# robertknight/rten

Measured on NVIDIA H100. Metric: resnet50_fp32_inferences_per_sec, higher is better.
Workload: dtype f32(tf32 mma, explicit opt-in)

## Files before the change

include/rten_b200.h:

```cpp
#ifndef RTEN_B200_H
#define RTEN_B200_H

#include <stddef.h>
#include <stdint.h>

#ifdef __cplusplus
extern "C" {
#endif

#define RTEN_MAX_DIMS 8
#define RTEN_DEVICE_HOST (-1)

typedef enum { RTEN_F32 = 0, RTEN_I32 = 1, RTEN_I8 = 2, RTEN_U8 = 3 } rten_dtype;

typedef struct {
    void* data;
    int32_t dtype;
    int32_t ndim;
    int64_t shape[RTEN_MAX_DIMS];
    int64_t strides[RTEN_MAX_DIMS];
    int32_t device;
    int32_t _reserved;
} rten_tensor;

// ... 37 lines not shown
rten_status rten_b200_ctx_create(int device, void* cuda_stream_or_null, size_t workspace_bytes, rten_ctx** out);
void rten_b200_ctx_destroy(rten_ctx* ctx);
const char* rten_b200_last_error(rten_ctx* ctx);
rten_status rten_b200_sync(rten_ctx* ctx);
rten_status rten_b200_set_f32_mode(rten_ctx* ctx, int mode );
rten_status rten_b200_set_autotune(rten_ctx* ctx, int enable);
rten_status rten_b200_save_plans(rten_ctx* ctx, const char* path);
rten_status rten_b200_load_plans(rten_ctx* ctx, const char* path);
rten_status rten_b200_alloc(rten_ctx* ctx, size_t bytes, void** dev_ptr);
rten_status rten_b200_free(rten_ctx* ctx, void* dev_ptr);
rten_status rten_b200_host_alloc(rten_ctx* ctx, size_t bytes, void** host_ptr);
rten_status rten_b200_host_free(rten_ctx* ctx, void* host_ptr);
rten_status rten_b200_copy(rten_ctx* ctx, const rten_tensor* src, rten_tensor* dst);
uint64_t rten_b200_launch_count(rten_ctx* ctx);
const char* rten_b200_version(void);
rten_status rten_b200_debug_forced_plans(rten_ctx* ctx, uint64_t* matched, uint64_t* unmatched);
typedef struct rten_graph rten_graph;
rten_status rten_b200_graph_begin(rten_ctx* ctx);
rten_status rten_b200_graph_end(rten_ctx* ctx, rten_graph** out);
rten_status rten_b200_graph_launch(rten_ctx* ctx, rten_graph* g);
void rten_b200_graph_destroy(rten_graph* g);

rten_status rten_b200_prepack_b(rten_ctx* ctx, const rten_tensor* b, rten_packed** out);
rten_status rten_b200_prepack_conv_weight(rten_ctx* ctx, const rten_tensor* w, int groups, rten_packed** out);
void rten_b200_packed_free(rten_ctx* ctx, rten_packed* p);

rten_status rten_b200_gemm(rten_ctx* ctx, const rten_tensor* a, const rten_tensor* b, const rten_tensor* c_or_null,
                           float alpha, float beta, int trans_a, int trans_b, rten_tensor* out);

rten_status rten_b200_matmul(rten_ctx* ctx, const rten_tensor* a, const rten_tensor* b,
                             const rten_packed* packed_b_or_null, const rten_tensor* row_bias_or_null, float alpha,
                             rten_tensor* out);
rten_status rten_b200_matmul_ex(rten_ctx* ctx, const rten_tensor* a, const rten_tensor* b,
                                const rten_packed* packed_b_or_null, const rten_tensor* row_bias_or_null, float alpha,
                                const rten_tensor* residual_or_null, int activation, rten_tensor* out);

rten_status rten_b200_matmul_integer(rten_ctx* ctx, const rten_tensor* a, const rten_tensor* b,
                                     const rten_packed* packed_b_or_null, const rten_tensor* a_zero_point_or_null,
                                     const rten_tensor* b_zero_point_or_null, const rten_tensor* scale_or_null,
                                     rten_tensor* out);
rten_status rten_b200_matmul_integer_ex(rten_ctx* ctx, const rten_tensor* a, const rten_tensor* b, const rten_packed* packed_b,
                                        const rten_tensor* a_zero_point, const rten_tensor* b_zero_point,
                                        const rten_tensor* scale, const rten_tensor* scale_b_or_null ,
                                        const rten_tensor* bias, const rten_tensor* residual, int activation,
                                        rten_tensor* out_range_or_null, rten_tensor* out);

rten_status rten_b200_matmul_nbits(rten_ctx* ctx, const rten_tensor* a, const rten_tensor* b, const rten_tensor* scales,
                                   int bits, int block_size, rten_tensor* out);

typedef struct {
    int32_t pads[4];
    int32_t auto_pad_same;
    int32_t groups;
    int32_t strides[2];
    int32_t dilations[2];
    int32_t n_strides;
    int32_t n_dilations;
} rten_conv_params;
rten_status rten_b200_conv2d(rten_ctx* ctx, const rten_tensor* x, const rten_tensor* w,
                             const rten_packed* packed_w_or_null, const rten_tensor* bias_or_null,
                             const rten_conv_params* p, rten_tensor* out);
rten_status rten_b200_conv2d_ex(rten_ctx* ctx, const rten_tensor* x, const rten_tensor* w,
                                const rten_packed* packed_w_or_null, const rten_tensor* bias_or_null,
                                const rten_conv_params* p, const rten_tensor* residual_or_null, int activation,
                                rten_tensor* out);
rten_status rten_b200_conv2d_act(rten_ctx* ctx, const rten_tensor* x, const rten_tensor* w,
                                 const rten_packed* packed_w_or_null, const rten_tensor* bias_or_null,
                                 const rten_conv_params* p, const rten_tensor* residual_or_null,
                                 const rten_activation* act_or_null, rten_tensor* out);
rten_status rten_b200_conv2d_projected(rten_ctx* ctx, const rten_tensor* x, const rten_tensor* w,
                                       const rten_packed* packed_w_or_null, const rten_tensor* bias_or_null,
                                       const rten_conv_params* p, const rten_tensor* x_proj, const rten_tensor* w_proj,
                                       const rten_packed* packed_w_proj_or_null, const rten_tensor* bias_proj_or_null,
                                       const rten_conv_params* p_proj, int activation, rten_tensor* out);
rten_status rten_b200_conv2d_chained(rten_ctx* ctx, const rten_tensor* x, const rten_tensor* w,
                                     const rten_packed* packed_w_or_null, const rten_tensor* bias_or_null,
                                     const rten_conv_params* p, const rten_tensor* residual_or_null,
                                     const rten_tensor* x_proj_or_null, const rten_tensor* w_proj_or_null,
                                     const rten_packed* packed_w_proj_or_null, const rten_tensor* bias_proj_or_null,
                                     const rten_conv_params* p_proj_or_null, int activation, const rten_tensor* w_next,
                                     const rten_packed* packed_w_next_or_null, const rten_tensor* bias_next_or_null,
                                     const rten_conv_params* p_next, int activation_next, rten_tensor* out,
                                     rten_tensor* out_next);
typedef struct {
    int32_t pads[4];
    int32_t auto_pad_same;
    int32_t groups;
    int32_t strides[2];
    int32_t dilations[2];
    int32_t output_padding[2];
    int32_t n_pads;
    int32_t n_strides;
    int32_t n_dilations;
    int32_t n_output_padding;
} rten_conv_transpose_params;
rten_status rten_b200_conv_transpose(rten_ctx* ctx, const rten_tensor* x, const rten_tensor* w,
                                     const rten_packed* packed_w_or_null, const rten_tensor* bias_or_null,
                                     const rten_conv_transpose_params* p, rten_tensor* out);
rten_status rten_b200_prepack_conv_transpose_weight(rten_ctx* ctx, const rten_tensor* w, const rten_conv_transpose_params* p,
                                                    rten_packed** out);
rten_status rten_b200_conv_integer(rten_ctx* ctx, const rten_tensor* x, const rten_tensor* w,
                                   const rten_packed* packed_w_or_null, const rten_tensor* x_zero_point_or_null,
                                   const rten_tensor* w_zero_point_or_null, const rten_tensor* scale_or_null,
                                   const rten_conv_params* p, rten_tensor* out);
rten_status rten_b200_conv_integer_ex(rten_ctx* ctx, const rten_tensor* x, const rten_tensor* w, const rten_packed* packed_w,
                                      const rten_tensor* x_zero_point, const rten_tensor* w_zero_point,
                                      const rten_tensor* scale, const rten_tensor* scale_b_or_null,
                                      const rten_conv_params* params, const rten_tensor* bias, const rten_tensor* residual,
                                      int activation, rten_tensor* out_range_or_null, rten_tensor* out);

rten_status rten_b200_quantized_linear(rten_ctx* ctx, const rten_tensor* x, const rten_tensor* ln_scale_or_null,
                                       const rten_tensor* ln_bias_or_null, float ln_epsilon, const rten_tensor* w,
                                       const rten_packed* packed_w_or_null, const rten_tensor* w_zero_point_or_null,
                                       const rten_tensor* w_scale, const rten_tensor* bias_or_null,
                                       const rten_tensor* residual_or_null, int activation, rten_tensor* out);
typedef struct {
    int32_t is_causal;
    int32_t q_num_heads;
    int32_t kv_num_heads;
    float scale;
    float softcap;
} rten_attention_params;
rten_status rten_b200_attention(rten_ctx* ctx, const rten_tensor* query, const rten_tensor* key, const rten_tensor* value,
                                const rten_tensor* attn_mask_or_null, const rten_tensor* nonpad_kv_seqlen_or_null,
                                const rten_attention_params* params, const rten_tensor* new_key_or_null,
                                const rten_tensor* new_value_or_null, rten_tensor* out);

rten_status rten_b200_rotary_embedding(rten_ctx* ctx, const rten_tensor* input, const rten_tensor* cos, const rten_tensor* sin,
                                       const rten_tensor* position_ids_or_null, int interleaved, int num_heads,
                                       int rotary_embedding_dim, rten_tensor* out);

typedef struct {
    int32_t num_heads;
    int32_t kv_num_heads;
    float scale;
    int32_t do_rotary;
    int32_t rotary_interleaved;
    int32_t local_window_size;
    float softcap;
} rten_gqa_params;
rten_status rten_b200_group_query_attention(rten_ctx* ctx, const rten_tensor* query, const rten_tensor* key_or_null,
                                            const rten_tensor* value_or_null, const rten_tensor* past_key_or_null,
                                            const rten_tensor* past_value_or_null, const rten_tensor* seqlens_k,
                                            const rten_tensor* total_sequence_length, const rten_tensor* cos_or_null,
                                            const rten_tensor* sin_or_null, const rten_tensor* position_ids_or_null,
                                            const rten_tensor* attention_bias_or_null, const rten_gqa_params* params,
                                            rten_tensor* out, rten_tensor* present_key, rten_tensor* present_value);

typedef struct {
    int32_t num_heads;
    float scale;
    float mask_filter_value;
    int32_t unidirectional;
} rten_mha_params;
rten_status rten_b200_multi_head_attention(rten_ctx* ctx, const rten_tensor* query, const rten_tensor* key_or_null,
                                           const rten_tensor* value_or_null, const rten_tensor* bias_or_null,
                                           const rten_tensor* key_padding_mask_or_null, const rten_tensor* attention_bias_or_null,
                                           const rten_tensor* past_key_or_null, const rten_tensor* past_value_or_null,
                                           const rten_tensor* past_sequence_length_or_null, const rten_tensor* cache_indirection_or_null,
                                           const rten_mha_params* params, rten_tensor* out, rten_tensor* present_key_or_null,
                                           rten_tensor* present_value_or_null);

typedef struct {
    int32_t direction;
    int32_t hidden_size;
    int32_t linear_before_reset;
// ... 112 lines not shown
```

rten_b200/_lib.py:

```python
from __future__ import annotations

import ctypes as C
import os

_HERE = os.path.dirname(os.path.abspath(__file__))
LIB_PATH = os.path.join(_HERE, "librten_b200.so")

RTEN_MAX_DIMS = 8
RTEN_DEVICE_HOST = -1
RTEN_F32, RTEN_I32, RTEN_I8, RTEN_U8 = 0, 1, 2, 3

STATUS_NAMES = {
    0: "Ok", 1: "CastFailed", 2: "UnsupportedType", 3: "IncompatibleInputShapes", 4: "MissingInputs",
    5: "InvalidValue", 6: "UnsupportedValue", 7: "UnsupportedOutput", 100: "Cuda", 101: "Nccl",
}


class RtenTensor(C.Structure):
    _fields_ = [
        ("data", C.c_void_p),
        ("dtype", C.c_int32),
        ("ndim", C.c_int32),
        ("shape", C.c_int64 * RTEN_MAX_DIMS),
        ("strides", C.c_int64 * RTEN_MAX_DIMS),
# ... 21 lines not shown
class RtenConvTransposeParams(C.Structure):
    _fields_ = [
        ("pads", C.c_int32 * 4),
        ("auto_pad_same", C.c_int32),
        ("groups", C.c_int32),
        ("strides", C.c_int32 * 2),
        ("dilations", C.c_int32 * 2),
        ("output_padding", C.c_int32 * 2),
        ("n_pads", C.c_int32),
        ("n_strides", C.c_int32),
        ("n_dilations", C.c_int32),
        ("n_output_padding", C.c_int32),
    ]


class RtenAttentionParams(C.Structure):
    _fields_ = [("is_causal", C.c_int32), ("q_num_heads", C.c_int32), ("kv_num_heads", C.c_int32), ("scale", C.c_float),
                ("softcap", C.c_float)]


class RtenGqaParams(C.Structure):
    _fields_ = [("num_heads", C.c_int32), ("kv_num_heads", C.c_int32), ("scale", C.c_float), ("do_rotary", C.c_int32),
                ("rotary_interleaved", C.c_int32), ("local_window_size", C.c_int32), ("softcap", C.c_float)]


class RtenMhaParams(C.Structure):
    _fields_ = [("num_heads", C.c_int32), ("scale", C.c_float), ("mask_filter_value", C.c_float), ("unidirectional", C.c_int32)]


class RtenActivation(C.Structure):
    _fields_ = [("kind", C.c_int32), ("alpha", C.c_float), ("beta", C.c_float)]


class RtenResizeParams(C.Structure):
    _fields_ = [("mode", C.c_int32), ("coord_mode", C.c_int32), ("nearest_mode", C.c_int32), ("n", C.c_int32),
                ("scales", C.c_float * 4), ("sizes", C.c_int64 * 4), ("use_sizes", C.c_int32)]


class RtenRnnParams(C.Structure):
    _fields_ = [("direction", C.c_int32), ("hidden_size", C.c_int32), ("linear_before_reset", C.c_int32)]


_TP = C.POINTER(RtenTensor)
_vp = C.c_void_p

_SIGNATURES = {
    "rten_b200_version": (C.c_char_p, []),
    "rten_b200_ctx_create": (C.c_int, [C.c_int, _vp, C.c_size_t, C.POINTER(_vp)]),
    "rten_b200_ctx_destroy": (None, [_vp]),
    "rten_b200_last_error": (C.c_char_p, [_vp]),
    "rten_b200_sync": (C.c_int, [_vp]),
    "rten_b200_set_f32_mode": (C.c_int, [_vp, C.c_int]),
    "rten_b200_set_autotune": (C.c_int, [_vp, C.c_int]),
    "rten_b200_save_plans": (C.c_int, [_vp, C.c_char_p]),
    "rten_b200_load_plans": (C.c_int, [_vp, C.c_char_p]),
    "rten_b200_alloc": (C.c_int, [_vp, C.c_size_t, C.POINTER(_vp)]),
    "rten_b200_free": (C.c_int, [_vp, _vp]),
    "rten_b200_host_alloc": (C.c_int, [_vp, C.c_size_t, C.POINTER(_vp)]),
    "rten_b200_host_free": (C.c_int, [_vp, _vp]),
    "rten_b200_copy": (C.c_int, [_vp, _TP, _TP]),
    "rten_b200_launch_count": (C.c_uint64, [_vp]),
    "rten_b200_debug_forced_plans": (C.c_int, [_vp, C.POINTER(C.c_uint64), C.POINTER(C.c_uint64)]),
    "rten_b200_graph_begin": (C.c_int, [_vp]),
    "rten_b200_graph_end": (C.c_int, [_vp, C.POINTER(_vp)]),
    "rten_b200_graph_launch": (C.c_int, [_vp, _vp]),
    "rten_b200_graph_destroy": (None, [_vp]),
    "rten_b200_prepack_b": (C.c_int, [_vp, _TP, C.POINTER(_vp)]),
    "rten_b200_prepack_conv_weight": (C.c_int, [_vp, _TP, C.c_int, C.POINTER(_vp)]),
    "rten_b200_packed_free": (None, [_vp, _vp]),
    "rten_b200_gemm": (C.c_int, [_vp, _TP, _TP, _TP, C.c_float, C.c_float, C.c_int, C.c_int, _TP]),
    "rten_b200_matmul": (C.c_int, [_vp, _TP, _TP, _vp, _TP, C.c_float, _TP]),
    "rten_b200_matmul_ex": (C.c_int, [_vp, _TP, _TP, _vp, _TP, C.c_float, _TP, C.c_int, _TP]),
    "rten_b200_matmul_integer": (C.c_int, [_vp, _TP, _TP, _vp, _TP, _TP, _TP, _TP]),
    "rten_b200_matmul_integer_ex": (C.c_int, [_vp, _TP, _TP, _vp, _TP, _TP, _TP, _TP, _TP, _TP, C.c_int, _TP, _TP]),
    "rten_b200_matmul_nbits": (C.c_int, [_vp, _TP, _TP, _TP, C.c_int, C.c_int, _TP]),
    "rten_b200_conv2d": (C.c_int, [_vp, _TP, _TP, _vp, _TP, C.POINTER(RtenConvParams), _TP]),
    "rten_b200_conv2d_ex": (C.c_int, [_vp, _TP, _TP, _vp, _TP, C.POINTER(RtenConvParams), _TP, C.c_int, _TP]),
    "rten_b200_conv2d_act": (C.c_int, [_vp, _TP, _TP, _vp, _TP, C.POINTER(RtenConvParams), _TP, C.POINTER(RtenActivation), _TP]),
    "rten_b200_conv2d_projected": (C.c_int, [_vp, _TP, _TP, _vp, _TP, C.POINTER(RtenConvParams), _TP, _TP, _vp, _TP,
                                             C.POINTER(RtenConvParams), C.c_int, _TP]),
    "rten_b200_conv2d_chained": (C.c_int, [_vp, _TP, _TP, _vp, _TP, C.POINTER(RtenConvParams), _TP, _TP, _TP, _vp, _TP,
                                           C.POINTER(RtenConvParams), C.c_int, _TP, _vp, _TP, C.POINTER(RtenConvParams),
                                           C.c_int, _TP, _TP]),
    "rten_b200_conv_transpose": (C.c_int, [_vp, _TP, _TP, _vp, _TP, C.POINTER(RtenConvTransposeParams), _TP]),
    "rten_b200_prepack_conv_transpose_weight": (C.c_int, [_vp, _TP, C.POINTER(RtenConvTransposeParams), C.POINTER(_vp)]),
    "rten_b200_conv_integer": (C.c_int, [_vp, _TP, _TP, _vp, _TP, _TP, _TP, C.POINTER(RtenConvParams), _TP]),
    "rten_b200_quantized_linear": (C.c_int, [_vp, _TP, _TP, _TP, C.c_float, _TP, _vp, _TP, _TP, _TP, _TP, C.c_int, _TP]),
    "rten_b200_attention": (C.c_int, [_vp, _TP, _TP, _TP, _TP, _TP, C.POINTER(RtenAttentionParams), _TP, _TP, _TP]),
    "rten_b200_rotary_embedding": (C.c_int, [_vp, _TP, _TP, _TP, _TP, C.c_int, C.c_int, C.c_int, _TP]),
    "rten_b200_group_query_attention": (C.c_int, [_vp, _TP, _TP, _TP, _TP, _TP, _TP, _TP, _TP, _TP, _TP, _TP,
                                                  C.POINTER(RtenGqaParams), _TP, _TP, _TP]),
    "rten_b200_multi_head_attention": (C.c_int, [_vp, _TP, _TP, _TP, _TP, _TP, _TP, _TP, _TP, _TP, _TP,
                                                 C.POINTER(RtenMhaParams), _TP, _TP, _TP]),
    "rten_b200_gru": (C.c_int, [_vp, _TP, _TP, _vp, _TP, _TP, _TP, _TP, C.POINTER(RtenRnnParams), _TP, _TP]),
    "rten_b200_lstm": (C.c_int, [_vp, _TP, _TP, _vp, _TP, _TP, _TP, _TP, _TP, _TP, C.POINTER(RtenRnnParams), _TP, _TP, _TP]),
    "rten_b200_softmax": (C.c_int, [_vp, _TP, _TP, C.c_int, C.c_int, _TP]),
    "rten_b200_layer_norm": (C.c_int, [_vp, _TP, _TP, _TP, C.c_int, C.c_float, _TP]),
    "rten_b200_rms_norm": (C.c_int, [_vp, _TP, _TP, C.c_int, C.c_float, _TP]),
    "rten_b200_skip_layer_norm": (C.c_int, [_vp, _TP, _TP, _TP, _TP, _TP, C.c_float, C.c_int, _TP, _TP]),
    "rten_b200_instance_norm": (C.c_int, [_vp, _TP, _TP, _TP, C.c_float, _TP]),
    "rten_b200_group_norm": (C.c_int, [_vp, _TP, C.c_int, _TP, _TP, _TP, _TP, C.c_float, C.POINTER(RtenActivation), _TP]),
    "rten_b200_erf": (C.c_int, [_vp, _TP, _TP]),
    "rten_b200_gelu": (C.c_int, [_vp, _TP, C.c_int, _TP]),
    "rten_b200_dynamic_quantize_linear": (C.c_int, [_vp, _TP, _TP, _TP, _TP, _vp]),
    "rten_b200_comm_unique_id": (C.c_int, [_vp]),
    "rten_b200_comm_create": (C.c_int, [_vp, _vp, C.c_int, C.c_int, C.POINTER(_vp)]),
    "rten_b200_comm_destroy": (None, [_vp]),
    "rten_b200_comm_uses_peer_memory": (C.c_int, [_vp]),
    "rten_b200_comm_timeouts": (C.c_int, [_vp]),
    "rten_b200_relu": (C.c_int, [_vp, _TP, _TP]),
    "rten_b200_sigmoid": (C.c_int, [_vp, _TP, _TP]),
    "rten_b200_silu": (C.c_int, [_vp, _TP, _TP]),
    "rten_b200_hard_sigmoid": (C.c_int, [_vp, _TP, C.c_float, C.c_float, _TP]),
    "rten_b200_hard_swish": (C.c_int, [_vp, _TP, _TP]),
    "rten_b200_clip": (C.c_int, [_vp, _TP, _TP, _TP, _TP]),
    "rten_b200_add": (C.c_int, [_vp, _TP, _TP, _TP]),
    "rten_b200_mul": (C.c_int, [_vp, _TP, _TP, _TP]),
    "rten_b200_sub": (C.c_int, [_vp, _TP, _TP, _TP]),
    "rten_b200_reduce_sum": (C.c_int, [_vp, _TP, C.POINTER(C.c_int32), C.c_int, C.c_int, _TP]),
    "rten_b200_conv_integer_ex": (C.c_int, [_vp, _TP, _TP, _vp, _TP, _TP, _TP, _TP, C.POINTER(RtenConvParams), _TP, _TP, C.c_int, _TP, _TP]),
    "rten_b200_range_reset": (C.c_int, [_vp, _TP]),
    "rten_b200_dynamic_quantize_linear_ranged": (C.c_int, [_vp, _TP, _TP, _TP, _TP, _TP, _vp]),
    "rten_b200_max_pool": (C.c_int, [_vp, _TP, C.POINTER(C.c_int32), C.POINTER(C.c_int32), C.POINTER(C.c_int32), _TP]),
    "rten_b200_global_average_pool": (C.c_int, [_vp, _TP, _TP]),
    "rten_b200_average_pool": (C.c_int, [_vp, _TP, C.POINTER(C.c_int32), C.POINTER(C.c_int32), C.POINTER(C.c_int32), C.c_int, _TP]),
    "rten_b200_resize": (C.c_int, [_vp, _TP, C.POINTER(RtenResizeParams), _TP]),
    "rten_b200_concat": (C.c_int, [_vp, C.POINTER(_TP), C.c_int, C.c_int, _TP]),
    "rten_b200_gather_rows": (C.c_int, [_vp, _TP, _TP, _TP]),
    "rten_b200_scatter_rows": (C.c_int, [_vp, _TP, _TP, _TP]),
    "rten_b200_model_load": (C.c_int, [_vp, _vp, C.c_size_t, C.POINTER(_vp)]),
    "rten_b200_model_free": (None, [_vp]),
    "rten_b200_model_num_inputs": (C.c_int32, [_vp]),
    "rten_b200_model_num_outputs": (C.c_int32, [_vp]),
    "rten_b200_model_input_name": (C.c_char_p, [_vp, C.c_int32]),
    "rten_b200_model_output_name": (C.c_char_p, [_vp, C.c_int32]),
    "rten_b200_model_num_nodes": (C.c_int32, [_vp]),
    "rten_b200_model_node_op": (C.c_char_p, [_vp, C.c_int32]),
    "rten_b200_model_summary": (C.c_char_p, [_vp]),
    "rten_b200_model_run": (C.c_int, [_vp, C.c_int32, C.POINTER(C.c_char_p), _TP, C.c_int32, C.POINTER(C.c_char_p), _TP]),
    "rten_b200_model_run_ex": (C.c_int, [_vp, C.c_int32, C.POINTER(C.c_char_p), _TP, C.c_void_p, C.c_int32, C.POINTER(C.c_char_p), _TP,
                                         C.POINTER(C.c_int32)]),
    "rten_b200_onnx_summary": (C.c_int, [_vp, C.c_size_t, C.c_char_p, C.c_size_t, C.POINTER(C.c_size_t)]),
}

_lib = None


def declared_symbols():
    return sorted(_SIGNATURES)


def load():
    global _lib
    if _lib is None:
        if not os.path.exists(LIB_PATH):
            raise RuntimeError(
                f"{LIB_PATH} is missing: run `python -c 'import __graft_entry__ as g; g.build()'` "
                "(rten_b200 has no CPU fallback)")
        lib = C.CDLL(LIB_PATH)
        for name, (res, args) in _SIGNATURES.items():
            fn = getattr(lib, name)
            fn.restype = res
            fn.argtypes = args
        _lib = lib
    return _lib
```

rten_b200/csrc/api_conv.cu:

```cuda
#include <cuda_runtime.h>

#include <algorithm>
#include <cstdlib>
#include <cstring>
#include <numeric>
#include <vector>

#include "api_shared.h"
#include "api_util.h"
#include "depthwise.h"
#include "resize.h"
#include "rowops.h"
#include "skinny.h"
#include "umma_gemm.h"

using namespace rtb;
using namespace rtb::api;

namespace {

struct ConvArgs {
    int kind;
    const rten_tensor* x;
    const rten_tensor* w;
    const rten_packed* pw;
    const rten_tensor* bias = nullptr;
    const rten_conv_params* p;
    const rten_tensor* residual = nullptr;
    int act = 0;
    float act_alpha = 0.0f, act_beta = 0.0f;
    const rten_tensor* x_zp = nullptr;
    const rten_tensor* w_zp = nullptr;
    const rten_tensor* scale = nullptr;
    const rten_tensor* scale_b = nullptr;
    const rten_tensor* out_range = nullptr;
    const void* x_lo = nullptr;
    bool cache_x3 = true;
};

rten_status pack_conv_weight(rten_ctx* ctx, const rten_tensor* w, int esize, void* dst) {
    const int64_t O = w->shape[0], Cg = w->shape[1], kh = w->shape[2], kw = w->shape[3];
    long long shape[4] = {O, kh, kw, Cg};
    long long ss[4] = {w->strides[0], w->strides[2], w->strides[3], w->strides[1]};
    long long ds[4] = {kh * kw * Cg, kw * Cg, Cg, 1};
    return launch_nd_copy(ctx, esize, w->data, dst, 4, shape, ss, ds);
}

void expand_1d(rten_tensor& t) {
    t.ndim = 4;
    t.shape[3] = t.shape[2];
    t.strides[3] = t.strides[2];
    t.shape[2] = 1;
    t.strides[2] = 0;
}

struct ConvShape {
    rten_tensor x, w, bias_v;
    bool one_d = false;
    int64_t strides[2], dil[2];
    int64_t B, C, H, W, O, Cg, kh, kw, OH, OW, pt, pb, pl, pr, Og;
    int groups;
};

rten_status conv_shape(OpScope& sc, const ConvArgs& A, ConvShape& S) {
    rten_ctx* ctx = sc.ctx;
    const rten_conv_params* cp = A.p;
    rten_tensor& x = S.x;
    rten_tensor& w = S.w;
    RTB_TRY(sc.in(A.x, &x));
    RTB_TRY(sc.in(A.w, &w));
    const bool one_d = S.one_d = x.ndim == 3;
    int64_t pads_in[4] = {cp->pads[0], cp->pads[1], cp->pads[2], cp->pads[3]};
    int64_t* strides = S.strides;
    int64_t* dil = S.dil;
    strides[0] = cp->strides[0];
    strides[1] = cp->strides[1];
    dil[0] = cp->dilations[0];
    dil[1] = cp->dilations[1];
    if (one_d) {
        if (w.ndim != 3) return fail(ctx, RTEN_ERR_INVALID_VALUE, "input must have 3 dims (OCW)");
        if (cp->n_strides != 1) return fail(ctx, RTEN_ERR_INVALID_VALUE, "expected 1 stride value");
        if (cp->n_dilations != 1) return fail(ctx, RTEN_ERR_INVALID_VALUE, "expected 1 dilation value");
        expand_1d(x);
        expand_1d(w);
        strides[1] = strides[0];
        strides[0] = 1;
        dil[1] = dil[0];
        dil[0] = 1;
        pads_in[1] = cp->pads[0];
        pads_in[3] = cp->pads[1];
        pads_in[0] = pads_in[2] = 0;
    } else {
        if (x.ndim != 4) return fail(ctx, RTEN_ERR_INVALID_VALUE, "input must have 4 dims (NCHW)");
        if (w.ndim != 4) return fail(ctx, RTEN_ERR_INVALID_VALUE, "input must have 4 dims (OCHW)");
        if (cp->n_strides != 2) return fail(ctx, RTEN_ERR_INVALID_VALUE, "expected 2 stride values");
        if (cp->n_dilations != 2) return fail(ctx, RTEN_ERR_INVALID_VALUE, "expected 2 dilation values");
    }
    S.B = x.shape[0];
    const int64_t C = S.C = x.shape[1], H = S.H = x.shape[2], W = S.W = x.shape[3];
    const int64_t O = S.O = w.shape[0], Cg = S.Cg = w.shape[1], kh = S.kh = w.shape[2], kw = S.kw = w.shape[3];
    if (A.bias) {
        RTB_TRY(sc.in(A.bias, &S.bias_v));
        if (S.bias_v.ndim != 1 || S.bias_v.shape[0] != O)
            return fail(ctx, RTEN_ERR_INCOMPATIBLE_SHAPES, "bias.size(0) != out_channels");
    }
    RTB_TRY(axis_out(ctx, H, kh, strides[0], cp->auto_pad_same != 0, pads_in[0], pads_in[2], dil[0], &S.OH, &S.pt, &S.pb));
    RTB_TRY(axis_out(ctx, W, kw, strides[1], cp->auto_pad_same != 0, pads_in[1], pads_in[3], dil[1], &S.OW, &S.pl, &S.pr));
    const int groups = S.groups = cp->groups;
    if (groups == 0) return fail(ctx, RTEN_ERR_INVALID_VALUE, "Group count must be > 0");
    if (groups < 0 || C % groups != 0) return fail(ctx, RTEN_ERR_INVALID_VALUE, "Input channel count not divisible by groups");
    if (C / groups != Cg)
        return fail(ctx, RTEN_ERR_INCOMPATIBLE_SHAPES, "Input channels (per group) does not match kernel input channels");
    if (O % groups != 0) return fail(ctx, RTEN_ERR_INVALID_VALUE, "Output channel count not divisible by groups");
    S.Og = O / groups;
    return RTEN_OK;
}

rten_status check_packed(rten_ctx* ctx, const ConvArgs& A, const ConvShape& S) {
    if (A.pw && (A.pw->kind != 1 || A.pw->O != S.O || A.pw->Cg != S.Cg || A.pw->kh != S.kh || A.pw->kw != S.kw))
        return fail(ctx, RTEN_ERR_INVALID_VALUE, "prepacked conv weight does not match the kernel shape");
// ... 67 lines not shown
    xs->strides[3] = C;
    return RTEN_OK;
}

OperandDesc nhwc(const rten_tensor& v, int64_t channels, int64_t off = 0) {
    OperandDesc d;
    d.base = (const uint8_t*)v.data + off * dtype_size(v.dtype);
    d.dims[0] = channels;
    d.dims[1] = v.shape[3];
    d.dims[2] = v.shape[2];
    d.dims[3] = v.shape[0];
    d.strides[1] = v.strides[3];
    d.strides[2] = v.strides[2];
    d.strides[3] = v.strides[0];
    return d;
}

OperandDesc packed_weight(const void* w, int64_t C, int64_t O, int64_t taps) {
    OperandDesc d;
    d.base = w;
    d.dims[0] = C;
    d.dims[1] = O;
    d.dims[2] = taps;
    d.strides[1] = taps * C;
    d.strides[2] = C;
    return d;
}

void conv_geom(GemmLaunch& L, const ConvShape& S) {
    L.conv = 1;
    L.M = (int)(S.B * S.OH * S.OW);
    L.N = (int)S.Og;
    L.K = (int)(S.kh * S.kw * S.Cg);
    ConvGeom& g = L.g;
    g.B = (int)S.B;
    g.H = (int)S.H;
    g.W = (int)S.W;
    g.C = (int)S.Cg;
    g.OH = (int)S.OH;
    g.OW = (int)S.OW;
    g.kh = (int)S.kh;
    g.kw = (int)S.kw;
    g.sy = (int)S.strides[0];
    g.sx = (int)S.strides[1];
    g.dy = (int)S.dil[0];
    g.dx = (int)S.dil[1];
    g.pt = (int)S.pt;
    g.pl = (int)S.pl;
}

void epi_out(EpilogueDesc& e, const rten_tensor& v, int64_t c0 = 0) {
    e.d = (uint8_t*)v.data + (size_t)(c0 * v.strides[1]) * 4;
    e.d_is_i32 = v.dtype == RTEN_I32;
    e.s_z0 = v.strides[0];
    e.s_row = v.strides[2];
    e.s_z1 = v.strides[3];
    e.s_col = v.strides[1];
}

void epi_residual(EpilogueDesc& e, const rten_tensor& r, int64_t c0 = 0) {
    e.r = (const float*)r.data + c0 * r.strides[1];
    e.r_scale = 1.0f;
    e.r_z0 = r.strides[0];
    e.r_row = r.strides[2];
    e.r_z1 = r.strides[3];
    e.r_col = r.strides[1];
}

rten_status conv_core(OpScope& sc, ConvArgs& A, rten_tensor* out) {
    rten_ctx* ctx = sc.ctx;
    ConvShape S;
    RTB_TRY(conv_shape(sc, A, S));
    const rten_tensor& x = S.x;
    const rten_tensor& w = S.w;
    const bool one_d = S.one_d;
    const int64_t* strides = S.strides;
    const int64_t* dil = S.dil;
    const int64_t B = S.B, C = S.C, H = S.H, W = S.W, O = S.O, Cg = S.Cg, kh = S.kh, kw = S.kw;
    const int64_t OH = S.OH, OW = S.OW, pt = S.pt, pb = S.pb, pl = S.pl, pr = S.pr, Og = S.Og;
    const int groups = S.groups;

    const int out_dtype = (A.kind == 1 && !A.scale) ? RTEN_I32 : RTEN_F32;
    rten_tensor ov;
    RTB_TRY(out_like(sc, out, out_dtype, x, one_d, B, O, OH, OW, &ov));
    if (B * O * OH * OW == 0) return RTEN_OK;

    const int esize = A.kind == 0 ? 4 : 1;
    RTB_TRY(check_packed(ctx, A, S));

    const bool x_signed = x.dtype == RTEN_I8, w_signed = w.dtype == RTEN_I8;
    rten_tensor xz_v{}, wz_v{};
    if (A.kind == 1) {
        if (A.x_zp) {
            RTB_TRY(sc.in(A.x_zp, &xz_v));
            if (numel(&xz_v) != 1) return fail(ctx, RTEN_ERR_INVALID_VALUE, "input zero point must be a scalar");
            if (xz_v.dtype != x.dtype) return fail(ctx, RTEN_ERR_CAST_FAILED, "zero point type does not match its tensor");
        }
        if (A.w_zp) {
            RTB_TRY(check_zero_point(ctx, A.w_zp, O, w.dtype));
            RTB_TRY(sc.in(A.w_zp, &wz_v));
        }
    }
    const float *scale_p = nullptr, *scale2_p = nullptr;
    if (A.scale) {
        rten_tensor s;
        RTB_TRY(sc.in(A.scale, &s));
        if (numel(&s) != 1 || s.ndim > 1) return fail(ctx, RTEN_ERR_INVALID_VALUE, "scale should be a scalar");
        scale_p = (const float*)s.data;
    }
    if (A.scale_b) {
        rten_tensor s;
        RTB_TRY(sc.in(A.scale_b, &s));
        if (s.dtype != RTEN_F32 || numel(&s) != 1) return fail(ctx, RTEN_ERR_INVALID_VALUE, "scale should be a scalar");
        scale2_p = (const float*)s.data;
    }
    int* range_p = nullptr;
    if (A.out_range) {
        if (A.out_range->dtype != RTEN_I32 || numel(A.out_range) != 2 || A.out_range->device < 0 || !is_contiguous(A.out_range))
            return fail(ctx, RTEN_ERR_INVALID_VALUE, "the output range must be a device-resident i32[2]");
        range_p = (int*)A.out_range->data;
    }
    rten_tensor res_v;
    if (A.residual) {
        RTB_TRY(sc.in(A.residual, &res_v));
        if (res_v.ndim != (one_d ? 3 : 4)) return fail(ctx, RTEN_ERR_INCOMPATIBLE_SHAPES, "residual shape does not match output");
        if (one_d) expand_1d(res_v);
        for (int i = 0; i < 4; i++)
            if (res_v.shape[i] != ov.shape[i]) return fail(ctx, RTEN_ERR_INCOMPATIBLE_SHAPES, "residual shape does not match output");
    }

    const bool pointwise_1x1 = kh == 1 && kw == 1 && (pt | pb | pl | pr) == 0 && groups == 1 && strides[0] == 1 &&
                               strides[1] == 1 && dil[0] == 1 && dil[1] == 1;
    if (C == O && groups == C && !pointwise_1x1) {
        DepthwiseParams d;
        d.x_dtype = x.dtype;
        d.w_dtype = w.dtype;
        d.B = (int)B;
        d.C = (int)C;
        d.H = (int)H;
        d.W = (int)W;
        d.OH = (int)OH;
        d.OW = (int)OW;
        d.kh = (int)kh;
        d.kw = (int)kw;
        d.sy = (int)strides[0];
        d.sx = (int)strides[1];
        d.dy = (int)dil[0];
        d.dx = (int)dil[1];
        d.pt = (int)pt;
        d.pl = (int)pl;
        d.x = x.data;
        d.out = ov.data;
        for (int i = 0; i < 4; i++) {
            d.xs[i] = x.strides[i];
            d.os[i] = ov.strides[i];
        }
        if (A.pw) {
            d.w = A.pw->data;
            d.ws_c = kh * kw;
            d.ws_h = kw;
            d.ws_w = 1;
        } else {
            d.w = w.data;
            d.ws_c = w.strides[0];
            d.ws_h = w.strides[2];
            d.ws_w = w.strides[3];
        }
        if (A.bias) {
            d.bias = (const float*)S.bias_v.data;
            d.bias_stride = S.bias_v.strides[0];
        }
        if (A.residual) {
            d.res = (const float*)res_v.data;
            for (int i = 0; i < 4; i++) d.rs[i] = res_v.strides[i];
        }
        d.act = A.act;
        d.act_alpha = A.act_alpha;
        d.act_beta = A.act_beta;
        if (A.kind == 1) {
            d.x_zp = A.x_zp ? xz_v.data : nullptr;
            d.w_zp = A.w_zp ? wz_v.data : nullptr;
            d.w_zp_stride = (A.w_zp && wz_v.ndim == 1) ? wz_v.strides[0] : 0;
            d.scale = scale_p;
            d.scale_b = scale2_p;
            d.range = range_p;
        }
        return launch_depthwise(ctx, d);
    }

    const void* wp = nullptr;
    const int32_t* w_colsum = nullptr;
    RTB_TRY(conv_weight(ctx, A, S, esize, &wp, &w_colsum));
    const uint8_t* za8 = nullptr;
    const int32_t* zb = nullptr;
    int zb_len = 0;
    int pad_value = 0;
    if (A.kind == 1) {
        pad_value = x_signed ? 0 : 128;
        if (A.x_zp) {
            za8 = (const uint8_t*)xz_v.data;
            if (!w_colsum) {
                int32_t* cs = nullptr;
                RTB_TRY(temp_alloc(ctx, (size_t)O * 4, (void**)&cs));
                RTB_TRY(launch_rowsum8(ctx, wp, w_signed, O, (int)(kh * kw * Cg), kh * kw * Cg, cs));
                w_colsum = cs;
            }
        }
        if (A.w_zp) {
            zb_len = wz_v.ndim == 0 ? 1 : (int)wz_v.shape[0];
            int32_t* p = nullptr;
            RTB_TRY(temp_alloc(ctx, (size_t)zb_len * 4, (void**)&p));
            RTB_TRY(launch_zp_to_i32(ctx, wz_v.data, w_signed, zb_len, wz_v.ndim == 0 ? 0 : wz_v.strides[0], p));
            zb = p;
        }
    }

// ... 4 lines not shown
        RTB_TRY(need_pad_copy ? nhwc_input(ctx, x, &xs, pt, pl, pb, pr, (uint8_t)pad_value) : nhwc_input(ctx, x, &xs));

    rten_tensor bias_c;
    if (A.bias) RTB_TRY(sc.contiguous(&S.bias_v, &bias_c));
    auto epilogue = [&](EpilogueDesc& e, int64_t c0) {
        epi_out(e, ov, c0);
        e.act = A.act;
        e.act_alpha = A.act_alpha;
        e.act_beta = A.act_beta;
        if (A.bias) {
            e.bias = (const float*)bias_c.data + c0;
            e.bias_kind = 1;
        }
        if (A.residual) epi_residual(e, res_v, c0);
        if (A.kind == 1) {
            e.za8 = za8;
            e.za8_signed = x_signed;
            e.scale2 = scale2_p;
            e.range = range_p;
            e.colsum = w_colsum ? w_colsum + c0 : nullptr;
            e.zb = zb ? (zb_len == 1 ? zb : zb + c0) : nullptr;
            e.zb_len = zb ? (zb_len == 1 ? 1 : (int)Og) : 0;
            e.scale = scale_p;
            e.scale_len = scale_p ? 1 : 0;
        }
    };

    const bool smallc_ok = !implicit_ok && groups == 1 && dil[1] == 1 && (int64_t)B * OH * OW > 0 &&
                           !getenv("RTEN_B200_NO_SMALLC") &&
                           (A.kind == 0 ? Cg <= 4 && kw * 4 <= 32 : Cg <= 16 && kw <= 8 && !zb);
    if (smallc_ok) {
        const bool q8 = A.kind == 1;
        const int64_t pitch = q8 ? 16 : 4, kb = 128 / esize;
        const int64_t Hp = q8 ? H + pt + pb : H;
        const int64_t Wp = std::max<int64_t>(q8 ? W + pl + pr : 0, (OW - 1) * strides[1] + 8);
        void *xp = nullptr, *wsm = nullptr;
        RTB_TRY(temp_alloc(ctx, (size_t)(B * Hp * Wp * pitch) * esize, &xp));
        if (q8) {
            RTB_TRY(launch_smallc8_pad(ctx, x.data, xp, (int)B, (int)C, (int)H, (int)W, (int)Hp, (int)Wp, (int)pt, (int)pl,
                                       x.strides[0], x.strides[1], x.strides[2], x.strides[3], pad_value));
        } else {
            RTB_TRY(launch_smallc_pad(ctx, (const float*)x.data, (float*)xp, (int)B, (int)C, (int)H, (int)W, (int)Wp, (int)pl,
                                      x.strides[0], x.strides[1], x.strides[2], x.strides[3]));
        }
        RTB_TRY(temp_alloc(ctx, (size_t)(O * kh * 128), &wsm));
        if (q8) {
            RTB_TRY(launch_smallc8_pack_w(ctx, w.data, wsm, (int)O, (int)C, (int)kh, (int)kw, w.strides[0], w.strides[1],
                                          w.strides[2], w.strides[3]));
        } else {
            RTB_TRY(launch_smallc_pack_w(ctx, (const float*)w.data, (float*)wsm, (int)O, (int)C, (int)kh, (int)kw, w.strides[0],
                                         w.strides[1], w.strides[2], w.strides[3]));
        }
        GemmLaunch L;
        L.kind = A.kind;
        L.a_signed = x_signed;
        L.b_signed = w_signed;
        conv_geom(L, S);
        L.K = (int)(kh * kb);
        L.g.H = (int)Hp;
        L.g.W = (int)OW;
        L.g.C = (int)kb;
        L.g.kw = 1;
        L.g.sx = 1;
        L.g.pt = q8 ? 0 : (int)pt;
        L.g.pl = 0;
        L.a.base = xp;
        L.a.dims[0] = kb;
        L.a.dims[1] = OW;
        L.a.dims[2] = Hp;
        L.a.dims[3] = B;
        L.a.strides[1] = strides[1] * pitch;
        L.a.strides[2] = Wp * pitch;
        L.a.strides[3] = Hp * Wp * pitch;
        if (!q8 && ctx->f32_mode == RTEN_F32_TF32X3 && !getenv("RTEN_B200_X3_THREE_PLANES")) {
            float* xlo = nullptr;
            const long long n = (long long)B * H * Wp * 4;
            RTB_TRY(temp_alloc(ctx, (size_t)n * 4, (void**)&xlo));
            const long long fd[4] = {n, 1, 1, 1}, fs[4] = {1, n, n, n};
            RTB_TRY(launch_tf32x3_split(ctx, (const float*)xp, xlo, fd, fs, n, 2));
            L.a_lo_base = xlo;
        }
        L.b = packed_weight(wsm, kb, O, kh);
        epilogue(L.epi, 0);
        const rten_status st = launch_umma_gemm(ctx, L);
        if (st != RTEN_ERR_UNSUPPORTED_VALUE) return st;
    }

    for (int g = 0; g < groups; g++) {
        GemmLaunch L;
        L.kind = A.kind;
        L.a_signed = x_signed;
        L.b_signed = w_signed;
        L.N = (int)Og;
        L.K = (int)(kh * kw * Cg);
        EpilogueDesc& e = L.epi;
        epilogue(e, g * Og);
        const uint8_t* wg = (const uint8_t*)wp + (size_t)(g * Og * kh * kw * Cg) * esize;

        if (implicit_ok) {
            conv_geom(L, S);
            L.g.H = (int)xs.shape[2];
            L.g.W = (int)xs.shape[3];
            if (need_pad_copy) L.g.pt = L.g.pl = 0;
            L.a = nhwc(xs, Cg, g * Cg);
            L.b = packed_weight(wg, Cg, Og, kh * kw);
            if (A.pw && A.kind == 0 && groups == 1 && wg == A.pw->data && A.cache_x3)
                L.b_x3_slot = &const_cast<rten_packed*>(A.pw)->x3;
            if (A.x_lo && xs.data == x.data) L.a_lo_base = (const float*)A.x_lo + g * Cg;
            if (zb) {
                int32_t* rs = nullptr;
                RTB_TRY(temp_alloc(ctx, (size_t)(B * OH * OW) * 4, (void**)&rs));
                void* ones = nullptr;
                RTB_TRY(temp_alloc(ctx, (size_t)(kh * kw * Cg), &ones));
                RTB_TRY(launch_fill8(ctx, ones, kh * kw * Cg, 1));
                GemmLaunch R = L;
                R.N = 1;
                R.b_signed = 1;
                R.b.base = ones;
                R.b.dims[1] = 1;
                R.epi = EpilogueDesc();
                R.epi.d = rs;
                R.epi.d_is_i32 = 1;
                R.epi.s_z0 = OH * OW;
                R.epi.s_row = OW;
                R.epi.s_z1 = 1;
                R.epi.s_col = B * OH * OW;
                if (const rten_status st = launch_umma_gemm(ctx, R)) return fail(ctx, st, "conv window-sum GEMM could not be launched");
                e.rowsum = rs;
            }
            const rten_status st = launch_umma_gemm(ctx, L);
            if (st != RTEN_ERR_UNSUPPORTED_VALUE) {
                RTB_TRY(st);
                continue;
            }
        }
        const int64_t Kd = kh * kw * Cg;
        const int64_t kpad = round_up(Kd, 16 / esize);
        void* col = nullptr;
        RTB_TRY(temp_alloc(ctx, (size_t)(B * OH * OW * kpad) * esize, &col));
        Im2ColParams ip;
        ip.B = (int)B;
        ip.C = (int)Cg;
        ip.H = (int)H;
        ip.W = (int)W;
        ip.OH = (int)OH;
        ip.OW = (int)OW;
        ip.kh = (int)kh;
        ip.kw = (int)kw;
        ip.sy = (int)strides[0];
        ip.sx = (int)strides[1];
        ip.dy = (int)dil[0];
        ip.dx = (int)dil[1];
        ip.pt = (int)pt;
        ip.pl = (int)pl;
        ip.c0 = (int)(g * Cg);
        ip.kpad = (int)kpad;
        ip.xs_b = x.strides[0];
        ip.xs_c = x.strides[1];
        ip.xs_h = x.strides[2];
        ip.xs_w = x.strides[3];
        RTB_TRY(launch_im2col(ctx, esize, x.data, col, ip, pad_value));
        L.conv = 0;
        L.M = (int)(B * OH * OW);
        L.z0 = L.z1 = 1;
        L.a = OperandDesc();
        L.a.base = col;
        L.a.dims[0] = Kd;
        L.a.dims[1] = B * OH * OW;
        L.a.strides[1] = kpad;
        L.b = OperandDesc();
        L.b.base = wg;
        L.b.dims[0] = Kd;
        L.b.dims[1] = Og;
        L.b.strides[1] = Kd;
        if (!tma_compatible(L.b, esize, 4)) {
            void* wb = nullptr;
            RTB_TRY(temp_alloc(ctx, (size_t)(Og * kpad) * esize, &wb));
            long long shape[2] = {Og, Kd}, ss[2] = {Kd, 1}, ds[2] = {kpad, 1};
            RTB_TRY(launch_nd_copy(ctx, esize, wg, wb, 2, shape, ss, ds));
            L.b.base = wb;
            L.b.strides[1] = kpad;
        }
        const bool uniform = (ov.strides[2] == OW * ov.strides[3]) && (ov.strides[0] == OH * ov.strides[2] || B == 1);
        const bool r_uniform = !A.residual || ((res_v.strides[2] == OW * res_v.strides[3]) &&
                                               (res_v.strides[0] == OH * res_v.strides[2] || B == 1));
        if (zb) {
            int32_t* rs = nullptr;
            RTB_TRY(temp_alloc(ctx, (size_t)(B * OH * OW) * 4, (void**)&rs));
            RTB_TRY(launch_rowsum8(ctx, col, x_signed, B * OH * OW, (int)Kd, kpad, rs));
            e.rowsum = rs;
        }
        if (uniform && r_uniform) {
            e.s_row = ov.strides[3];
            e.s_z0 = e.s_z1 = 0;
            if (A.residual) {
                e.r_row = res_v.strides[3];
                e.r_z0 = e.r_z1 = 0;
            }
            if (const rten_status st = launch_umma_gemm(ctx, L)) return fail(ctx, st, "conv GEMM could not be launched");
        } else {
            void* tmp = nullptr;
            RTB_TRY(temp_alloc(ctx, (size_t)(B * OH * OW * Og) * 4, &tmp));
            EpilogueDesc e2 = e;
            e2.d = tmp;
            e2.s_row = Og;
            e2.s_col = 1;
            e2.s_z0 = e2.s_z1 = 0;
            e2.r = nullptr;
            e2.act = A.residual ? 0 : A.act;
            GemmLaunch L2 = L;
            L2.epi = e2;
            if (const rten_status st = launch_umma_gemm(ctx, L2)) return fail(ctx, st, "conv GEMM could not be launched");
            long long shape[4] = {B, OH, OW, Og};
            long long ss[4] = {OH * OW * Og, OW * Og, Og, 1};
            long long ds[4] = {ov.strides[0], ov.strides[2], ov.strides[3], ov.strides[1]};
            if (A.residual) {
                long long rs4[4] = {res_v.strides[0], res_v.strides[2], res_v.strides[3], res_v.strides[1]};
// ... 614 lines not shown
    p->kh = S.kh;
    p->kw = S.kw;
    p->groups = S.groups;
    p->sy = S.sy;
    p->sx = S.sx;
    p->dy = S.dy;
    p->dx = S.dx;
    p->phases.assign((size_t)(S.sy * S.sx), nullptr);
    for (int64_t ry = 0; ry < S.sy; ry++)
        for (int64_t rx = 0; rx < S.sx; rx++) {
            const AxisTaps ty = axis_taps(S.kh, S.sy, S.dy, ry), tx = axis_taps(S.kw, S.sx, S.dx, rx);
            if (ty.T == 0 || tx.T == 0) continue;
            rten_packed* ph = new rten_packed();
            p->phases[(size_t)(ry * S.sx + rx)] = ph;
            ph->kind = 1;
            ph->O = S.O;
            ph->Cg = S.Cg;
            ph->kh = ty.T;
            ph->kw = tx.T;
            ph->groups = S.groups;
            RTB_TRY(pool_alloc(ctx, (size_t)std::max<int64_t>(S.O * ty.T * tx.T * S.Cg, 1) * 4, &ph->data));
            RTB_TRY(pack_transpose_phase(ctx, S, ty, tx, ph->data));
        }
    RTB_TRY(sc.finish(RTEN_OK));
    *out = p.release();
    return RTEN_OK;
}

rten_status rten_b200_conv_transpose(rten_ctx* ctx, const rten_tensor* x, const rten_tensor* w, const rten_packed* pw,
                                     const rten_tensor* bias, const rten_conv_transpose_params* p, rten_tensor* out) {
    RTB_TRY(check_ctx(ctx));
    if (!x || !w || !p || !out) return fail(ctx, RTEN_ERR_MISSING_INPUTS, "missing inputs");
    if (x->dtype != RTEN_F32 || w->dtype != RTEN_F32 || (bias && bias->dtype != RTEN_F32))
        return fail(ctx, RTEN_ERR_UNSUPPORTED_TYPE, "unsupported type");
    OpScope sc(ctx);
    return sc.finish(conv_transpose_core(sc, x, w, pw, bias, p, out));
}

rten_status rten_b200_conv2d(rten_ctx* ctx, const rten_tensor* x, const rten_tensor* w, const rten_packed* pw,
                             const rten_tensor* bias, const rten_conv_params* p, rten_tensor* out) {
    return rten_b200_conv2d_ex(ctx, x, w, pw, bias, p, nullptr, 0, out);
}

rten_status rten_b200_conv_integer(rten_ctx* ctx, const rten_tensor* x, const rten_tensor* w, const rten_packed* pw,
                                   const rten_tensor* x_zp, const rten_tensor* w_zp, const rten_tensor* scale,
                                   const rten_conv_params* p, rten_tensor* out) {
    return rten_b200_conv_integer_ex(ctx, x, w, pw, x_zp, w_zp, scale, nullptr, p, nullptr, nullptr, 0, nullptr, out);
}

rten_status rten_b200_conv_integer_ex(rten_ctx* ctx, const rten_tensor* x, const rten_tensor* w, const rten_packed* pw,
                                      const rten_tensor* x_zp, const rten_tensor* w_zp, const rten_tensor* scale,
                                      const rten_tensor* scale_b, const rten_conv_params* p, const rten_tensor* bias,
                                      const rten_tensor* residual, int activation, rten_tensor* out_range,
                                      rten_tensor* out) {
    RTB_TRY(check_ctx(ctx));
    if (!x || !w || !p || !out) return fail(ctx, RTEN_ERR_MISSING_INPUTS, "missing inputs");
    auto is8 = [](int dt) { return dt == RTEN_U8 || dt == RTEN_I8; };
    if (!is8(x->dtype) || !is8(w->dtype)) return fail(ctx, RTEN_ERR_UNSUPPORTED_TYPE, "unsupported type");
    if (scale && scale->dtype != RTEN_F32) return fail(ctx, RTEN_ERR_CAST_FAILED, "scale must be float");
    if ((bias || residual || activation || scale_b) && !scale)
        return fail(ctx, RTEN_ERR_INVALID_VALUE, "bias / residual / activation follow the float conversion: a scale is required");
    if ((bias && bias->dtype != RTEN_F32) || (residual && residual->dtype != RTEN_F32))
        return fail(ctx, RTEN_ERR_UNSUPPORTED_TYPE, "unsupported type");
    if (activation < 0 || activation > 1) return fail(ctx, RTEN_ERR_UNSUPPORTED_VALUE, "only Relu can follow an integer convolution");
    if (out_range && !scale) return fail(ctx, RTEN_ERR_INVALID_VALUE, "the output range is defined for float outputs: a scale is required");
    OpScope sc(ctx);
    ConvArgs A{};
    A.kind = 1;
    A.x = x;
    A.w = w;
    A.pw = (pw && pw->dtype == w->dtype) ? pw : nullptr;
    A.p = p;
    A.x_zp = x_zp;
    A.w_zp = w_zp;
    A.scale = scale;
    A.scale_b = scale_b;
    A.bias = bias;
    A.residual = residual;
    A.act = activation;
    A.out_range = out_range;
    return sc.finish(conv_core(sc, A, out));
}

static rten_status pool2d(rten_ctx* ctx, const rten_tensor* x, const int32_t kernel[2], const int32_t pads[4],
                          const int32_t strides[2], bool average, int count_include_pad, rten_tensor* out) {
    RTB_TRY(check_ctx(ctx));
    if (!x || !out) return fail(ctx, RTEN_ERR_MISSING_INPUTS, "missing inputs");
    if (x->dtype != RTEN_F32) return fail(ctx, RTEN_ERR_UNSUPPORTED_TYPE, "unsupported type");
    if (x->ndim != 4) return fail(ctx, RTEN_ERR_INVALID_VALUE, "input must have 4 dims (NCHW)");
    OpScope sc(ctx);
    rten_tensor xv, ov;
    RTB_TRY(sc.in(x, &xv));
    int64_t OH = 0, OW = 0, p0, p1;
    RTB_TRY(axis_out(ctx, xv.shape[2], kernel[0], strides[0], false, pads[0], pads[2], 1, &OH, &p0, &p1));
    RTB_TRY(axis_out(ctx, xv.shape[3], kernel[1], strides[1], false, pads[1], pads[3], 1, &OW, &p0, &p1));
    const int64_t B = xv.shape[0], C = xv.shape[1];
    RTB_TRY(out_like(sc, out, RTEN_F32, xv, false, B, C, OH, OW, &ov));
    PoolParams p;
    p.B = (int)B;
    p.C = (int)C;
    p.H = (int)xv.shape[2];
    p.W = (int)xv.shape[3];
    p.OH = (int)OH;
    p.OW = (int)OW;
    p.kh = kernel[0];
    p.kw = kernel[1];
    p.sy = strides[0];
    p.sx = strides[1];
    p.pt = pads[0];
    p.pl = pads[1];
    p.xs_b = xv.strides[0];
    p.xs_c = xv.strides[1];
    p.xs_h = xv.strides[2];
    p.xs_w = xv.strides[3];
    p.ys_b = ov.strides[0];
    p.ys_c = ov.strides[1];
    p.ys_h = ov.strides[2];
    p.ys_w = ov.strides[3];
    p.channels_fastest = ov.strides[1] == 1;
    return sc.finish(average ? launch_avgpool(ctx, (const float*)xv.data, (float*)ov.data, p, count_include_pad)
                             : launch_maxpool(ctx, (const float*)xv.data, (float*)ov.data, p));
}

rten_status rten_b200_max_pool(rten_ctx* ctx, const rten_tensor* x, const int32_t kernel[2], const int32_t pads[4],
                               const int32_t strides[2], rten_tensor* out) {
    return pool2d(ctx, x, kernel, pads, strides, false, 0, out);
}

rten_status rten_b200_average_pool(rten_ctx* ctx, const rten_tensor* x, const int32_t kernel[2], const int32_t pads[4],
                                   const int32_t strides[2], int count_include_pad, rten_tensor* out) {
    return pool2d(ctx, x, kernel, pads, strides, true, count_include_pad, out);
}

rten_status rten_b200_resize(rten_ctx* ctx, const rten_tensor* x, const rten_resize_params* p, rten_tensor* out) {
    RTB_TRY(check_ctx(ctx));
    if (!x || !p || !out) return fail(ctx, RTEN_ERR_MISSING_INPUTS, "missing inputs");
    if (x->dtype != RTEN_F32) return fail(ctx, RTEN_ERR_UNSUPPORTED_TYPE, "unsupported type");
    if (p->mode < RTEN_RESIZE_NEAREST || p->mode > RTEN_RESIZE_LINEAR || p->coord_mode < RTEN_RESIZE_HALF_PIXEL ||
        p->coord_mode > RTEN_RESIZE_PYTORCH_HALF_PIXEL || p->nearest_mode < RTEN_RESIZE_FLOOR ||
        p->nearest_mode > RTEN_RESIZE_ROUND_PREFER_CEIL)
        return fail(ctx, RTEN_ERR_INVALID_VALUE, "unknown resize mode");
    OpScope sc(ctx);
    rten_tensor xv;
    RTB_TRY(sc.in(x, &xv));
    const int nd = xv.ndim;
    int64_t osz[4] = {0, 0, 0, 0};
    float inv[4] = {1.0f, 1.0f, 1.0f, 1.0f};
    RTB_TRY(resize_output_size(ctx, xv, p, osz, inv));
    bool same = true;
    for (int i = 0; i < nd; i++) same = same && osz[i] == xv.shape[i];
    auto eq = [&](int i) { return osz[i] == xv.shape[i]; };
    int map[4] = {-1, -1, -1, -1};
    if (same) {
    } else if (nd == 4 && eq(0) && eq(1)) {
        map[0] = 0, map[1] = 1, map[2] = 2, map[3] = 3;
    } else if (nd == 3 && eq(0) && eq(1)) {
        map[0] = 0, map[1] = 1, map[3] = 2;
    } else if (nd == 3 && eq(0)) {
        map[0] = 0, map[2] = 1, map[3] = 2;
    } else if (nd == 2) {
        map[2] = 0, map[3] = 1;
    } else if (nd == 1) {
        map[3] = 0;
    } else {
        return fail(ctx, RTEN_ERR_UNSUPPORTED_VALUE, "Only 1D to 4D inputs are supported with up to two resized dimensions");
    }
    rten_tensor ov;
    RTB_TRY(nd == 4 ? out_like(sc, out, RTEN_F32, xv, false, osz[0], osz[1], osz[2], osz[3], &ov)
                    : sc.out(out, RTEN_F32, nd, osz, &ov, nullptr));
    if (same) return sc.finish(numel(&xv) ? copy_view(ctx, xv, ov) : RTEN_OK);
    ResizeParams r;
    r.mode = p->mode;
    r.coord_mode = p->coord_mode;
    r.nearest_mode = p->nearest_mode;
    int64_t in4[4], out4[4];
    for (int i = 0; i < 4; i++) {
        const int a = map[i];
        in4[i] = a >= 0 ? xv.shape[a] : 1;
        out4[i] = a >= 0 ? osz[a] : 1;
        r.xs[i] = a >= 0 ? xv.strides[a] : 0;
        r.os[i] = a >= 0 ? ov.strides[a] : 0;
    }
    if (out4[0] * out4[1] * out4[2] * out4[3] != 0 && in4[2] * in4[3] == 0)
        return fail(ctx, RTEN_ERR_INVALID_VALUE, "cannot resize an empty input");
    for (int i = 0; i < 4; i++)
        if (in4[i] > INT32_MAX || out4[i] > INT32_MAX) return fail(ctx, RTEN_ERR_UNSUPPORTED_VALUE, "dimension too large");
    r.B = (int)out4[0];
    r.C = (int)out4[1];
    r.H = (int)in4[2];
    r.W = (int)in4[3];
    r.OH = (int)out4[2];
    r.OW = (int)out4[3];
    r.inv_y = map[2] >= 0 ? inv[map[2]] : 1.0f;
    r.inv_x = inv[map[3]];
    r.x = (const float*)xv.data;
    r.out = (float*)ov.data;
    return sc.finish(launch_resize(ctx, r));
}

rten_status rten_b200_concat(rten_ctx* ctx, const rten_tensor* const* inputs, int n, int axis, rten_tensor* out) {
    RTB_TRY(check_ctx(ctx));
    if (!inputs || n < 1 || !out) return fail(ctx, RTEN_ERR_MISSING_INPUTS, "missing inputs");
    for (int i = 0; i < n; i++)
        if (!inputs[i]) return fail(ctx, RTEN_ERR_MISSING_INPUTS, "missing inputs");
// ... 133 lines not shown
```

rten_b200/csrc/umma_epilogue.cuh:

```cuda
#pragma once

namespace rtb {

struct RowPos {
    bool ok;
    int z0, z1, y, m;
};

__device__ __forceinline__ RowPos decode_row(const KParams& p, const TileCoord& tc, int r) {
    RowPos w;
    if (p.conv) {
        int xi, r2, yi, bi;
        p.d_tw.divmod(r, r2, xi);
        p.d_th.divmod(r2, bi, yi);
        w.z0 = tc.b0 + bi;
        w.z1 = tc.ox0 + xi;
        w.y = tc.oy0 + yi;
        w.ok = (bi < p.tb) && (w.z1 < p.OW) && (w.y < p.OH) && (w.z0 < p.Bn);
        w.m = (w.z0 * p.OH + w.y) * p.OW + w.z1;
    } else {
        w.z0 = tc.z0;
        w.z1 = tc.z1;
        w.y = w.m = tc.m0 + r;
        w.ok = w.m < p.M;
// ... 275 lines not shown
    float s2;
    unsigned zc = 0;
    float sc = 0.0f, bv = 0.0f;
    int col;
    __device__ PlainI8Epi(const KParams& p, const SmemLayout& L, int grp)
        : zc_s(reinterpret_cast<unsigned*>(L.bias) + grp * 128), scl_s(L.bias + 256 + grp * 128),
          bias_s(L.bias + 512 + grp * 128),
          za_v(p.epi.za8 ? (unsigned)(p.epi.za8_signed ? (int)(int8_t)__ldg(p.epi.za8) : (int)__ldg(p.epi.za8)) : 0u),
          s2(p.epi.scale2 ? __ldg(p.epi.scale2) : 1.0f),
          col(((threadIdx.x & 127) >> 5) * 64 + grp * 32 + (threadIdx.x & 31)) {}

    __device__ __forceinline__ void unit(const KParams& p, int t) {
        const TileCoord tc = decode_tile(p, t);
        const EpilogueDesc& e = p.epi;
        const int n = tc.n0 + col;
        zc = 0;
        sc = bv = 0.0f;
        if (col < p.bn && n < p.N) {
            if (e.za8) zc = za_v * (unsigned)__ldg(e.colsum + n);
            sc = e.scale_len == 1 ? __ldg(e.scale) : __ldg(e.scale + n);
            if (e.scale2) sc = __fmul_rn(s2, sc);
            if (e.bias_kind == 1) bv = __ldg(e.bias + n);
        }
    }
    __device__ __forceinline__ void ready(int grp) {
        const int i = threadIdx.x & 127;
        zc_s[i] = zc;
        scl_s[i] = sc;
        bias_s[i] = bv;
        group_sync(grp);
    }
    __device__ __forceinline__ void row(const KParams& p, const TileCoord& tc, int r) {
        row_ok = !p.epi.range || decode_row(p, tc, r).ok;
    }

    __device__ __forceinline__ void math(const KParams& p, uint32_t (&v)[32], int k, int nbase, uint8_t* rowp, int sw) {
        const EpilogueDesc& e = p.epi;
        if (nbase >= p.N) return;
        const uint4* zq = reinterpret_cast<const uint4*>(zc_s + 32 * k);
        const float4* sq = reinterpret_cast<const float4*>(scl_s + 32 * k);
        const float4* bq = reinterpret_cast<const float4*>(bias_s + 32 * k);
#pragma unroll
        for (int j = 0; j < 32; j += 4) {
            const uint4 z = zq[j >> 2];
            const float4 s4 = sq[j >> 2];
            uint32_t f0 = __float_as_uint(__int2float_rn((int)(v[j] - z.x)));
            uint32_t f1 = __float_as_uint(__int2float_rn((int)(v[j + 1] - z.y)));
            uint32_t f2 = __float_as_uint(__int2float_rn((int)(v[j + 2] - z.z)));
            uint32_t f3 = __float_as_uint(__int2float_rn((int)(v[j + 3] - z.w)));
            mul_f32x2(f0, f1, s4.x, s4.y);
            mul_f32x2(f2, f3, s4.z, s4.w);
            if (e.bias_kind == 1) {
                const float4 bb = bq[j >> 2];
                add_f32x2(f0, f1, bb.x, bb.y);
                add_f32x2(f2, f3, bb.z, bb.w);
            }
            if (p.res_tma) {
                const float4 rr = *reinterpret_cast<const float4*>(staged_chunk(rowp, sw, j >> 2));
                add_f32x2(f0, f1, rr.x, rr.y);
                add_f32x2(f2, f3, rr.z, rr.w);
            }
            if (e.act == 1) {
                f0 = __float_as_uint(fmaxf(__uint_as_float(f0), 0.0f));
                f1 = __float_as_uint(fmaxf(__uint_as_float(f1), 0.0f));
                f2 = __float_as_uint(fmaxf(__uint_as_float(f2), 0.0f));
                f3 = __float_as_uint(fmaxf(__uint_as_float(f3), 0.0f));
            }
            if (GELU) act4_bits(f0, f1, f2, f3, e);
            v[j] = f0;
            v[j + 1] = f1;
            v[j + 2] = f2;
            v[j + 3] = f3;
        }
        if (e.range && row_ok) {
#pragma unroll
            for (int j = 0; j < 32; j += 2) {
                rg_lo = fminf(rg_lo, fminf(__uint_as_float(v[j]), __uint_as_float(v[j + 1])));
                rg_hi = fmaxf(rg_hi, fmaxf(__uint_as_float(v[j]), __uint_as_float(v[j + 1])));
            }
        }
    }
};

template <int KIND, Epi E>
using EpiOps = std::conditional_t<E == Epi::Generic, GenericEpi<KIND>,
               std::conditional_t<E == Epi::Fast || E == Epi::FastGelu, FastEpi<KIND, E == Epi::FastGelu>,
               std::conditional_t<E == Epi::PlainF32 || E == Epi::PlainF32Gelu, PlainF32Epi<E == Epi::PlainF32Gelu>,
                                  PlainI8Epi<E == Epi::PlainI8Gelu>>>>;

template <int KIND, Epi E>
__device__ __forceinline__ void epilogue(const KParams& p, const SmemLayout& L, const CUtensorMap* tma_d,
                                         const CUtensorMap* tma_r, int worker, int n_workers) {
    using Ops = EpiOps<KIND, E>;
    const EpilogueDesc& e = p.epi;
    const int warp = threadIdx.x >> 5, lane = threadIdx.x & 31;
    const int q = warp & 3;
    const int grp = (warp - 4) >> 2;
    const int r = q * 32 + lane;
    const int sw = r & 7;
    const int nbuf = p.nbuf;
    uint8_t* const stg0 = L.smem + (size_t)p.stages * p.stage_bytes + grp * nbuf * STG_BYTES;
    const bool issuer = (q == 0 && lane == 0);
    const int splitk = Ops::kSplitK ? p.splitk : 1;
    const bool tma_store = Ops::kDirectStore ? p.tma_store != 0 : true;
    Ops ops(p, L, grp);
    uint32_t ci = 0;
    uint32_t aphase = 0, rphase = 0;
    for (int u = worker, it = 0; u < p.units_total; u += n_workers, it++) {
        int t = u, ks = 0;
        if (splitk > 1) p.d_tiles_total.divmod(u, ks, t);
        const int acc = it & 1;
        auto request_residual = [&](const TileCoord& tc, uint32_t c, int col, int in_flight) {
            const int b = c % nbuf;
            bulk_wait_read(in_flight);
            uint64_t* rb = &L.res_bar[grp * 4 + b];
            mbar_expect_tx(rb, p.res_tx_bytes);
            const int4 x = out_coord(p, tc, col);
            tma_load_4d(stg0 + b * STG_BYTES, tma_r, rb, x.x, x.y, x.z, x.w);
        };
        const bool first_res = p.res_tma && issuer && grp * 32 < p.bn;
        if (first_res && splitk == 1) request_residual(decode_tile(p, t), ci, grp * 32, nbuf - 1);
        const TileCoord tc0 = decode_tile(p, t);
        ops.unit(p, t);
        mbar_wait(&L.acc_full[acc], (aphase >> acc) & 1);
        aphase ^= 1u << acc;
        ops.ready(grp);
        const uint32_t t_row = ((uint32_t)(q * 32) << 16) + acc * ACC_STRIDE;
        bool owner = true;
        if (splitk > 1) {
            owner = splitk_publish(p, t, ks, grp, q, lane, t_row, &L.sk_flag[grp], L.acc_smem);
            if (owner && first_res) request_residual(decode_tile(p, t), ci, grp * 32, nbuf - 1);
        }
        if (owner) {
            const TileCoord tc = (E == Epi::Fast || E == Epi::FastGelu) ? tc0 : decode_tile(p, t);
            ops.row(p, tc, r);
            if (const int c0 = grp * 32, k = 0; c0 < p.bn) {
                uint32_t v[32];
                if (splitk > 1)
                    splitk_sum<KIND>(p, t, c0, r, v);
                else
                    acc_ld(L.acc_smem, t_row + c0, v);
                const int nbase = tc.n0 + c0;
                const int bcur = ci % nbuf;
                uint8_t* stg = stg0 + bcur * STG_BYTES;
                uint8_t* rowp = stg + r * 128;
                if (p.res_tma) {
                    mbar_wait(&L.res_bar[grp * 4 + bcur], (rphase >> bcur) & 1);
                    rphase ^= 1u << bcur;
                }
                ops.math(p, v, k, nbase, rowp, sw);
                if (tma_store && nbuf == 1) {
                    if (issuer) bulk_wait_read(0);
                    group_sync(grp);
                }
#pragma unroll
                for (int j = 0; j < 8; j++)
                    *reinterpret_cast<uint4*>(staged_chunk(rowp, sw, j)) = make_uint4(v[4 * j], v[4 * j + 1], v[4 * j + 2], v[4 * j + 3]);
                ops.staged(p, nbase, rowp, sw);
                if (tma_store) {
                    if (issuer && !p.res_tma && nbuf > 1) bulk_wait_read(nbuf - 2);
                    fence_proxy_async();
                    group_sync(grp);
                    if (issuer) {
                        const int4 x = out_coord(p, tc, c0);
                        tma_store_4d(tma_d, stg, x.x, x.y, x.z, x.w);
                        asm volatile("cp.async.bulk.commit_group;" ::: "memory");
                    }
                } else if (ops.row_ok) {
                    if constexpr (Ops::kDirectStore) {
                        uint32_t* dptr = reinterpret_cast<uint32_t*>(e.d) + ops.d_off;
#pragma unroll 1
                        for (int j = 0; j < 32 && nbase + j < p.N; j++)
                            dptr[(long long)(nbase + j) * e.s_col] = *staged_word(rowp, sw, j);
                    }
                }
                ci++;
            }
        }
        __syncwarp();
        if (lane == 0) mbar_arrive(&L.acc_empty[acc]);
    }
    ops.finish(e);
    if (tma_store && issuer) asm volatile("cp.async.bulk.wait_group.read 0;" ::: "memory");
}

}
```

rten_b200/csrc/umma_gemm.cu:

```cuda
#include <cuda.h>
#include <cuda_runtime.h>

#include <algorithm>
#include <array>
#include <cmath>
#include <vector>
#include <cmath>
#include <cstdint>
#include <cstdio>
#include <cstdlib>

#include "math.cuh"
#include "ptx.cuh"
#include "rowops.h"
#include "umma_gemm.h"
#include "umma_kernel.cuh"

namespace rtb {

typedef CUresult (*EncodeTiledFn)(CUtensorMap*, CUtensorMapDataType, cuuint32_t, void*, const cuuint64_t*,
                                  const cuuint64_t*, const cuuint32_t*, const cuuint32_t*, CUtensorMapInterleave,
                                  CUtensorMapSwizzle, CUtensorMapL2promotion, CUtensorMapFloatOOBfill);

static EncodeTiledFn get_encode(rten_ctx* ctx) {
// ... 12 lines not shown
    if (reinterpret_cast<uintptr_t>(od.base) & 15) return false;
    if (od.strides[0] != 1) return false;
    for (int i = 1; i < rank; i++) {
        if (od.dims[i] > 1) {
            if ((od.strides[i] * esize) % 16 != 0) return false;
            if (od.strides[i] * esize >= (1ll << 40)) return false;
        }
    }
    for (int i = 0; i < rank; i++)
        if (od.dims[i] < 1 || od.dims[i] > 0xFFFFFFFFll) return false;
    return true;
}

bool encode_map(rten_ctx* ctx, CUtensorMap* map, const OperandDesc& od, int esize, bool is_f32,
                const uint32_t box[4], const uint32_t estr[4]) {
    EncodeTiledFn enc = get_encode(ctx);
    if (!enc) return false;
    cuuint64_t dims[4];
    cuuint64_t strides[3];
    cuuint32_t b[4], es[4];
    for (int i = 0; i < 4; i++) {
        dims[i] = (cuuint64_t)od.dims[i];
        b[i] = box[i];
        es[i] = estr[i];
    }
    for (int i = 1; i < 4; i++) {
        long long s = od.strides[i] * esize;
        if (s == 0 || od.dims[i] == 1) s = 16;
        strides[i - 1] = (cuuint64_t)s;
    }
    CUresult r = enc(map, is_f32 ? CU_TENSOR_MAP_DATA_TYPE_FLOAT32 : CU_TENSOR_MAP_DATA_TYPE_UINT8, 4,
                     const_cast<void*>(od.base), dims, strides, b, es, CU_TENSOR_MAP_INTERLEAVE_NONE,
                     CU_TENSOR_MAP_SWIZZLE_128B, CU_TENSOR_MAP_L2_PROMOTION_L2_256B,
                     CU_TENSOR_MAP_FLOAT_OOB_FILL_NONE);
    return r == CUDA_SUCCESS;
}

static void pick_conv_tile(const ConvGeom& g, int& tw, int& th, int& tb) {
    double best = -1.0;
    tw = th = tb = 1;
    for (int w = 1; w <= std::min(g.OW, 128); w++) {
        if (w * g.sx > 256) break;
        for (int h = 1; h <= std::min(g.OH, 128 / w); h++) {
            if (h * g.sy > 256) break;
            int b = std::min(g.B, 128 / (w * h));
            if (b < 1) continue;
            long long tiles = (long long)((g.OW + w - 1) / w) * ((g.OH + h - 1) / h) * ((g.B + b - 1) / b);
            double eff = (double)g.B * g.OH * g.OW / ((double)tiles * 128.0);
            if (eff > best + 1e-9 || (eff > best - 1e-9 && w > tw)) {
                best = eff;
                tw = w;
                th = h;
                tb = b;
            }
        }
    }
}

struct Plan {
    int bn = 32, splitk = 1, nbuf = 1;
    bool halo = false;
    int T = 0;
};

static Plan halo_plan(int bn, int T) {
    Plan pl;
    pl.halo = true;
    pl.bn = bn;
    pl.T = T;
    return pl;
}

struct Prepared {
    KParams p;
    uint32_t abox[4], aes[4], bbox_k;
    uint32_t pbox[4], pes[4];
    uint32_t a_rows;
    long long batch;
    OperandDesc od, ord;
    uint32_t dbox[4];
    int tma_store, res_tma;
    int wide;
    int chain_bytes;
    int step;
    int esize, kelems;
};

constexpr int SK_CNT_INTS = 1 << 16;
static int smem_budget_for(int n_stg) { return 227 * 1024 - SMEM_FIXED_BYTES - n_stg * STG_BYTES; }
static int wide_stages(int stage_bytes, int chain_bytes) {
    return std::min(MAX_STAGES, (227 * 1024 - WIDE_SMEM_FIXED_BYTES - chain_bytes) / stage_bytes);
}
static bool is_wide(int bn) { return bn > ACC_STRIDE; }

static Epi pick_epilogue(const GemmLaunch& L, int tma_store, int res_tma, int splitk) {
    const EpilogueDesc& e = L.epi;
    auto aligned = [](const void* ptr) { return (reinterpret_cast<uintptr_t>(ptr) & 15) == 0; };
    bool fast = tma_store && (L.N % 32) == 0 && !getenv("RTEN_B200_NO_FAST") && e.bias_kind != 2 &&
                (e.r == nullptr || res_tma) && (e.bias_kind != 1 || aligned(e.bias));
    if (L.kind == 1)
        fast = fast && (!(e.za || e.za8) || aligned(e.colsum)) && (!e.zb || e.zb_len == 1 || (e.zb_len == L.N && aligned(e.zb))) &&
               (!e.scale || e.scale_len == 1 || (e.scale_len == L.N && aligned(e.scale)));
    if (!fast) return Epi::Generic;
    const bool gelu = e.act > 1;
    if (!getenv("RTEN_B200_NO_PLAIN") && e.act <= 7) {
        if (L.kind == 0 && e.alpha == 1.0f && !e.range && (e.r == nullptr || e.r_scale == 1.0f))
            return gelu ? Epi::PlainF32Gelu : Epi::PlainF32;
        if (L.kind == 1 && e.scale && !e.za && !e.zb && (e.scale_len == 1 || e.scale_len == L.N) && splitk == 1 &&
            (!e.za8 || e.colsum))
            return gelu ? Epi::PlainI8Gelu : Epi::PlainI8;
    }
    return gelu ? Epi::FastGelu : Epi::Fast;
}

static const char* epi_name(Epi v) {
    static const char* const names[] = {"Generic", "Fast", "FastGelu", "PlainF32", "PlainF32Gelu", "PlainI8", "PlainI8Gelu"};
    return names[(int)v];
}

static bool is_plain_f32(Epi v) { return v == Epi::PlainF32 || v == Epi::PlainF32Gelu; }

struct PlanShape {
    long long tiles_n, units_m, tiles, units;
    int kb_per, stage_bytes, stages, n_stg;
};

static bool plan_shape(const Prepared& q, const Plan& pl, PlanShape& ps) {
    const KParams& p = q.p;
    if (pl.splitk < 1) return false;
    if (is_wide(pl.bn)) {
        if ((pl.bn != 128 && pl.bn != 256) || !q.wide || pl.splitk != 1) return false;
        if (pl.bn == 256 && q.p.epi.act > 1) return false;
    } else if (pl.bn < 16 || pl.bn % 32 || pl.bn % q.step) {
        return false;
    }
    if (pl.nbuf < (q.res_tma ? 2 : 1) || pl.nbuf > 4) return false;
    ps.tiles_n = q.chain_bytes ? 1 : (p.N + pl.bn - 1) / pl.bn;
    ps.units_m = p.tiles_m;
    ps.tiles = ps.units_m * ps.tiles_n * q.batch;
    ps.units = ps.tiles * pl.splitk;
    if (ps.units > 0x7FFFFFFFll) return false;
    ps.kb_per = (p.k_blocks + pl.splitk - 1) / pl.splitk;
    if (pl.splitk > 1) {
        if (pl.bn % 32 || (long long)(pl.splitk - 1) * ps.kb_per >= p.k_blocks) return false;
        if (ps.tiles * 2 > SK_CNT_INTS) return false;
    }
    ps.n_stg = 2 * pl.nbuf;
    ps.stage_bytes = A_STAGE_BYTES + pl.bn * KBYTES;
    ps.stages = is_wide(pl.bn) ? wide_stages(ps.stage_bytes, q.chain_bytes) : std::min(MAX_STAGES, smem_budget_for(ps.n_stg) / ps.stage_bytes);
    if (ps.stages < 2) return false;
    return true;
}

static double plan_cost(const Prepared& q, const Plan& pl, const PlanShape& ps, int num_sms) {
    const double active = (double)std::min<long long>(ps.units, num_sms);
    const double waves = std::ceil((double)ps.units / num_sms);
    const double bw = std::min(64.0, 7400.0 / active);
    const double mmas = 4.0;
    const double t_kb = std::max(mmas * std::max(42.0, (double)pl.bn), ps.stage_bytes / bw);
    double t_stage = std::max(t_kb, 320.0 + mmas * 42.0);
    t_stage = std::max(t_stage, 2300.0 / ps.stages);
    const double mainloop = ps.kb_per * t_stage;
    const double epi = is_wide(pl.bn) ? (pl.bn / 32.0) * 400.0 + 600.0 : (pl.bn / 32.0) * 350.0 / 2.0 + 600.0;
    double unit = (is_wide(pl.bn) ? mainloop + epi : std::max(mainloop, epi)) + 1500.0;
    double cost = waves * unit + 2500.0;
    if (pl.splitk > 1) cost += epi * (1.0 + 0.25 * pl.splitk) + 1500.0;

    return cost;
}

static void enumerate_plans(const Prepared& q, int num_sms, std::vector<std::pair<double, Plan>>& out) {
    const KParams& p = q.p;
    const int nmax = (p.N + q.step - 1) / q.step * q.step;
    static const int splits[] = {1, 2, 3, 4, 5, 6, 8, 10, 12, 16};
    for (int bn : {32, 64, 128, 256}) {
        if (bn > nmax && bn != 32) break;
        for (int sk : splits) {
            Plan pl;
            pl.bn = bn;
            pl.splitk = sk;
            if (sk > 1 && p.k_blocks / sk < 4) continue;
            const int kb_per = (p.k_blocks + sk - 1) / sk;
            pl.nbuf = (q.res_tma || kb_per < 24) ? 2 : 1;
            PlanShape ps;
            if (is_wide(bn)) {
                pl.nbuf = 2;
            } else if (pl.nbuf == 2 && !getenv("RTEN_B200_NO_NBUF3")) {
                PlanShape ps2;
                const bool ok2 = plan_shape(q, pl, ps2);
                pl.nbuf = 3;
                if (!plan_shape(q, pl, ps) || (ps.stages < 3 && !(ok2 && ps.stages == ps2.stages))) pl.nbuf = 2;
            }
            if (!plan_shape(q, pl, ps)) continue;
            if (sk > 1 && ps.tiles >= 2 * num_sms) continue;
            if (ps.stages < 2) continue;
            out.emplace_back(plan_cost(q, pl, ps, num_sms), pl);
        }
    }
    std::sort(out.begin(), out.end(), [](const std::pair<double, Plan>& x, const std::pair<double, Plan>& y) {
        return x.first < y.first;
    });
}

static rten_status prepare_launch(rten_ctx* ctx, const GemmLaunch& L, Prepared& q) {
    const int esize = L.kind == 0 ? 4 : 1;
    const int kelems = KBYTES / esize;
    if (!tma_compatible(L.a, esize, 4) || !tma_compatible(L.b, esize, 4)) return RTEN_ERR_UNSUPPORTED_VALUE;
    if (L.M <= 0 || L.N <= 0 || L.K <= 0) return RTEN_ERR_UNSUPPORTED_VALUE;
    q.esize = esize;
    q.kelems = kelems;
    KParams& p = q.p;
    memset(&p, 0, sizeof(p));
    p.M = L.M;
    p.N = L.N;
    p.K = L.K;
    p.z0 = L.z0;
    p.z1 = L.z1;
    p.kelems = kelems;
    p.conv = L.conv;
    p.epi = L.epi;
    p.c_blocks = 1;
    p.kw = 1;
    for (int i = 0; i < 4; i++) q.aes[i] = 1;
    if (L.conv) {
        const ConvGeom& g = L.g;
        pick_conv_tile(g, p.tw, p.th, p.tb);
        p.tiles_x = (g.OW + p.tw - 1) / p.tw;
        p.tiles_y = (g.OH + p.th - 1) / p.th;
        int tiles_b = (g.B + p.tb - 1) / p.tb;
        p.tiles_m = p.tiles_x * p.tiles_y * tiles_b;
        p.OH = g.OH;
        p.OW = g.OW;
        p.Bn = g.B;
        p.sy = g.sy;
        p.sx = g.sx;
        p.dy = g.dy;
        p.dx = g.dx;
        p.pt = g.pt;
        p.pl = g.pl;
        p.kw = g.kw;
        p.c_blocks = (g.C + kelems - 1) / kelems;
        p.k_blocks = g.kh * g.kw * p.c_blocks;
        p.z0 = p.z1 = 1;
        q.abox[0] = kelems;
        q.abox[1] = p.tw * g.sx;
        q.abox[2] = p.th * g.sy;
        q.abox[3] = p.tb;
        q.aes[1] = g.sx;
        q.aes[2] = g.sy;
        q.a_rows = p.tw * p.th * p.tb;
        q.batch = 1;
    } else {
        p.tiles_m = (L.M + BM - 1) / BM;
        p.k_blocks = (L.K + kelems - 1) / kelems;
        q.abox[0] = kelems;
        q.abox[1] = BM;
        q.abox[2] = 1;
        q.abox[3] = 1;
        q.a_rows = BM;
        q.batch = (long long)L.z0 * L.z1;
        p.a_bcast0 = (L.a.dims[2] == 1 && L.z0 > 1) ? 1 : 0;
        p.a_bcast1 = (L.a.dims[3] == 1 && L.z1 > 1) ? 1 : 0;
        p.b_bcast0 = (L.b.dims[2] == 1 && L.z0 > 1) ? 1 : 0;
        p.b_bcast1 = (L.b.dims[3] == 1 && L.z1 > 1) ? 1 : 0;
    }
    OperandDesc& od = q.od;
    OperandDesc& ord = q.ord;
    q.dbox[0] = 32;
    q.dbox[1] = q.dbox[2] = q.dbox[3] = 1;
    const EpilogueDesc& e = L.epi;
    od.base = e.d;
    od.dims[0] = L.N;
    od.strides[0] = 1;
    if (L.conv) {
        od.dims[1] = L.g.OW;
        od.dims[2] = L.g.OH;
        od.dims[3] = L.g.B;
        od.strides[1] = e.s_z1;
        od.strides[2] = e.s_row;
        od.strides[3] = e.s_z0;
        q.dbox[1] = p.tw;
        q.dbox[2] = p.th;
        q.dbox[3] = p.tb;
    } else {
        od.dims[1] = L.M;
        od.dims[2] = L.z0;
        od.dims[3] = L.z1;
        od.strides[1] = e.s_row;
        od.strides[2] = e.s_z0;
        od.strides[3] = e.s_z1;
        q.dbox[1] = BM;
    }
    q.tma_store = (e.s_col == 1 && L.N >= 4 && tma_compatible(od, 4, 4)) ? 1 : 0;
    if (getenv("RTEN_B200_NO_TMA_STORE")) q.tma_store = 0;
    ord = od;
    ord.base = e.r;
    if (L.conv) {
        ord.strides[1] = e.r_z1;
        ord.strides[2] = e.r_row;
        ord.strides[3] = e.r_z0;
    } else {
        ord.strides[1] = e.r_row;
        ord.strides[2] = e.r_z0;
        ord.strides[3] = e.r_z1;
    }
    q.res_tma = (q.tma_store && (L.kind == 0 || e.scale) && e.r && e.r_col == 1 && (L.N % 32) == 0 &&
                 (e.bias_kind != 1 || (reinterpret_cast<uintptr_t>(e.bias) & 15) == 0) && tma_compatible(ord, 4, 4))
                    ? 1
                    : 0;
    for (int i = 1; i < 4; i++)
        if (ord.dims[i] > 1 && ord.strides[i] == 0) q.res_tma = 0;
    if (getenv("RTEN_B200_NO_RES_TMA")) q.res_tma = 0;
    p.res_tx_bytes = q.a_rows * KBYTES;
    q.step = q.tma_store ? 32 : 16;
    const bool plain = is_plain_f32(pick_epilogue(L, q.tma_store, q.res_tma, 1));
    q.wide = plain && !getenv("RTEN_B200_NO_WIDE");
    p.kb_main = p.k_blocks;
    if (L.proj.C > 0) {
        const GemmLaunch::Projection& pr = L.proj;
        const int s = pr.stride;
        if (!L.conv || L.kind != 0 || pr.C % kelems || s < 1 || s > 8 || p.tw * s > 256 || p.th * s > 256 || !plain ||
            pr.a.dims[0] * (pr.x3_cb ? 3 : 1) != pr.C || pr.b.dims[0] != pr.C || !tma_compatible(pr.a, 4, 4) || !tma_compatible(pr.b, 4, 4))
            return RTEN_ERR_UNSUPPORTED_VALUE;
        p.kb_proj = pr.C / kelems;
        p.s_proj = s;
        p.k_blocks += p.kb_proj;
        const uint32_t box[4] = {(uint32_t)kelems, (uint32_t)(p.tw * s), (uint32_t)(p.th * s), (uint32_t)p.tb};
        const uint32_t es[4] = {1, (uint32_t)s, (uint32_t)s, 1};
        for (int i = 0; i < 4; i++) {
            q.pbox[i] = box[i];
            q.pes[i] = es[i];
        }
    }
    q.chain_bytes = 0;
    if (L.chain.N2 > 0) {
        const GemmLaunch::Chain& c = L.chain;
        if (!L.conv || L.kind != 0 || ctx->f32_mode != RTEN_F32_TF32 || !q.wide || !q.tma_store || L.epi.act > 1 ||
            L.N % 32 || L.N > 256 || (c.N2 != 64 && c.N2 != 128) || c.act < 0 || c.act > 1 || c.w.dims[0] != L.N ||
            c.w.dims[1] != c.N2 || c.z.dims[0] != c.N2 || !tma_compatible(c.w, 4, 4) || !tma_compatible(c.z, 4, 4) ||
            (L.epi.r && !q.res_tma))
            return RTEN_ERR_UNSUPPORTED_VALUE;
        q.chain_bytes = L.N / 32 * c.N2 * KBYTES;
    }
    return RTEN_OK;
}

static size_t splitk_ws_bytes(const PlanShape& ps, const Plan& pl) {
    return pl.splitk > 1 ? (size_t)ps.tiles * pl.splitk * (pl.bn / 32) * 4096 * 4 : 0;
}

static rten_status ensure_splitk_counters(rten_ctx* ctx) {
    if (!ctx->sk_counters) {
        cudaError_t ce = cudaMalloc(&ctx->sk_counters, SK_CNT_INTS * sizeof(int));
        if (ce != cudaSuccess) return fail_cuda(ctx, ce, "split-K counters");
        ce = cudaMemset(ctx->sk_counters, 0, SK_CNT_INTS * sizeof(int));
        if (ce != cudaSuccess) return fail_cuda(ctx, ce, "split-K counters");
    }
    return RTEN_OK;
}

static rten_status launch_plan(rten_ctx* ctx, const GemmLaunch& L, const Prepared& q, const Plan& pl, bool verbose,
                               void* ws = nullptr) {
    PlanShape ps;
    if (!plan_shape(q, pl, ps)) return RTEN_ERR_UNSUPPORTED_VALUE;
    KParams p = q.p;
    p.bn = pl.bn;
    p.splitk = pl.splitk;
    p.nbuf = pl.nbuf;
    p.tma_store = q.tma_store;
    p.res_tma = q.res_tma ? 1 : 0;
    p.kb_per = ps.kb_per;
    p.tiles_n = (int)ps.tiles_n;
    p.tiles_total = (int)ps.tiles;
    p.units_total = (int)ps.units;
    p.d_tiles_n.set(p.tiles_n);
    p.d_tiles_m.set(p.tiles_m);
    p.d_z0.set(p.z0);
    p.d_tiles_x.set(p.conv ? p.tiles_x : 1);
    p.d_tiles_y.set(p.conv ? p.tiles_y : 1);
    p.d_tiles_total.set(p.tiles_total);
    p.d_c_blocks.set(p.c_blocks);
    p.d_kw.set(p.kw);
    p.d_tw.set(p.conv ? p.tw : 1);
    p.d_th.set(p.conv ? p.th : 1);
    p.stage_bytes = ps.stage_bytes;
    p.tx_bytes = q.a_rows * KBYTES + p.bn * KBYTES;
    p.stages = ps.stages;
    p.sgn = L.kind == 0 ? 0 : (L.a_signed ? 1 : 0) | (L.b_signed ? 2 : 0);
    if (p.splitk > 1) {
        RTB_TRY(ensure_splitk_counters(ctx));
        if (!ws) RTB_TRY(temp_alloc(ctx, splitk_ws_bytes(ps, pl), &ws));
        p.sk_ws = reinterpret_cast<uint32_t*>(ws);
        p.sk_cnt = reinterpret_cast<int*>(ctx->sk_counters);
    }

    uint32_t bbox[4] = {(uint32_t)q.kelems, (uint32_t)p.bn, 1, 1}, bes[4] = {1, 1, 1, 1}, des[4] = {1, 1, 1, 1};
    TmaMaps m;
    if (!encode_map(ctx, &m.a, L.a, q.esize, L.kind == 0, q.abox, q.aes)) return RTEN_ERR_UNSUPPORTED_VALUE;
    if (!encode_map(ctx, &m.b, L.b, q.esize, L.kind == 0, bbox, bes)) return RTEN_ERR_UNSUPPORTED_VALUE;
    m.d = m.r = m.a2 = m.a_proj = m.b_proj = m.a2_proj = m.w2 = m.z = m.a;
    p.x3_cb = L.x3_cb;
    if (L.x3_cb && !encode_map(ctx, &m.a2, L.a_lo, q.esize, true, q.abox, q.aes)) return RTEN_ERR_UNSUPPORTED_VALUE;
    if (p.kb_proj) {
        p.x3_cb_proj = L.proj.x3_cb;
        if (!encode_map(ctx, &m.a_proj, L.proj.a, 4, true, q.pbox, q.pes) ||
            !encode_map(ctx, &m.b_proj, L.proj.b, 4, true, bbox, bes) ||
            (L.proj.x3_cb && !encode_map(ctx, &m.a2_proj, L.proj.a_lo, 4, true, q.pbox, q.pes)))
            return RTEN_ERR_UNSUPPORTED_VALUE;
    }
    if (p.tma_store && !encode_map(ctx, &m.d, q.od, 4, true, q.dbox, des)) {
        p.tma_store = 0;
        p.res_tma = 0;
        m.d = m.a;
    }
    if (p.res_tma && !encode_map(ctx, &m.r, q.ord, 4, true, q.dbox, des)) {
        p.res_tma = 0;
        m.r = m.a;
    }
    const Epi epi = pick_epilogue(L, p.tma_store, p.res_tma, p.splitk);
    if (epi == Epi::Generic && (L.kind == 1 || L.epi.act > 1)) p.res_tma = 0;
    if (q.chain_bytes) {
        const GemmLaunch::Chain& c = L.chain;
        const uint32_t wbox[4] = {32, (uint32_t)c.N2, 1, 1}, zbox[4] = {32, q.dbox[1], q.dbox[2], q.dbox[3]};
        if (epi != Epi::PlainF32 || (L.epi.r && !p.res_tma) || !encode_map(ctx, &m.w2, c.w, 4, true, wbox, des) ||
            !encode_map(ctx, &m.z, c.z, 4, true, zbox, des))
            return RTEN_ERR_UNSUPPORTED_VALUE;
        p.chain_n2 = c.N2;
        p.chain_passes = (L.N + p.bn - 1) / p.bn;
        p.chain_act = c.act;
        p.chain_bias = c.bias;
    }

    if (verbose)
        fprintf(stderr, "[umma_gemm] kind=%d conv=%d M=%d N=%d K=%d kb=%d kb_proj=%d tiles_m=%d bn=%d splitk=%d units=%d stages=%d tma_store=%d res_tma=%d nbuf=%d box=%dx%dx%d epi=%s%s\n",
                L.kind, L.conv, L.M, L.N, L.K, p.k_blocks, p.kb_proj, p.tiles_m, p.bn, p.splitk, p.units_total, p.stages,
                p.tma_store, p.res_tma, p.nbuf, p.tw, p.th, p.tb, epi_name(epi),
                p.chain_n2 == 64 ? " chain=64" : p.chain_n2 == 128 ? " chain=128" : "");
    if ((is_wide(p.bn) || p.kb_proj || L.epi.bias2) && !is_plain_f32(epi)) return RTEN_ERR_UNSUPPORTED_VALUE;
    const size_t smem_bytes = (size_t)p.stages * p.stage_bytes + q.chain_bytes +
                              (is_wide(p.bn) ? WIDE_SMEM_FIXED_BYTES : ps.n_stg * STG_BYTES + SMEM_FIXED_BYTES);
    using Kernel = void (*)(TmaMaps, KParams);
    static const Kernel narrow[2][7] = {
        {umma_gemm_kernel<0, Epi::Generic>, umma_gemm_kernel<0, Epi::Fast>, umma_gemm_kernel<0, Epi::FastGelu>,
         umma_gemm_kernel<0, Epi::PlainF32>, umma_gemm_kernel<0, Epi::PlainF32Gelu>, nullptr, nullptr},
        {umma_gemm_kernel<1, Epi::Generic>, umma_gemm_kernel<1, Epi::Fast>, umma_gemm_kernel<1, Epi::FastGelu>, nullptr,
         nullptr, umma_gemm_kernel<1, Epi::PlainI8>, umma_gemm_kernel<1, Epi::PlainI8Gelu>}};
    const Kernel kern = !is_wide(p.bn)              ? narrow[L.kind][(int)epi]
                        : p.chain_n2 == 64         ? umma_wide_kernel<Epi::PlainF32, 64>
                        : p.chain_n2 == 128        ? umma_wide_kernel<Epi::PlainF32, 128>
                        : epi == Epi::PlainF32Gelu ? umma_wide_kernel<Epi::PlainF32Gelu>
                                                   : umma_wide_kernel<Epi::PlainF32>;

    const int threads = is_wide(p.bn) ? WIDE_THREADS : NUM_THREADS;
    return launch(ctx, "umma_gemm launch", kern, {std::min(p.units_total, ctx->num_sms), threads, smem_bytes, 227 * 1024, true}, m, p);
}

static std::vector<long long> tune_key(const GemmLaunch& L, const Prepared& q) {
    const EpilogueDesc& e = L.epi;
    std::vector<long long> k = {L.kind, L.conv, L.M, L.N, L.K, L.z0, L.z1, q.tma_store, q.res_tma, e.act, e.bias_kind,
                                e.r != nullptr, (e.za != nullptr || e.za8 != nullptr), e.zb != nullptr, e.scale != nullptr,
                                L.a.strides[1], L.b.strides[1], L.x3_cb};
    if (L.conv) {
        const ConvGeom& g = L.g;
        for (long long v : {g.B, g.H, g.W, g.C, g.OH, g.OW, g.kh, g.kw, g.sy, g.sx, g.dy, g.dx, g.pt, g.pl}) k.push_back(v);
    }
    if (L.proj.C > 0) {
        const GemmLaunch::Projection& pr = L.proj;
        for (int64_t v : {(int64_t)-1, (int64_t)pr.C, (int64_t)pr.stride, (int64_t)pr.x3_cb, pr.a.dims[1], pr.a.dims[2],
                          pr.a.strides[1], pr.a.strides[2], pr.a.strides[3], pr.b.strides[1]})
            k.push_back(v);
    }
    return k;
}

static std::array<int, 3> plan_record(const Plan& pl) {
    return pl.halo ? std::array<int, 3>{-1, pl.bn, pl.T} : std::array<int, 3>{pl.bn, pl.splitk, pl.nbuf};
}

static Plan plan_from_record(const std::array<int, 3>& r) {
    if (r[0] < 0) return halo_plan(r[1], r[2]);
    Plan pl;
    pl.bn = r[0];
    pl.splitk = r[1];
    pl.nbuf = r[2];
    return pl;
}

void tune_cache_load(rten_ctx* ctx, const char* path) {
    FILE* f = fopen(path, "r");
    if (!f) return;
    char line[2048];
    while (fgets(line, sizeof(line), f)) {
        std::vector<long long> key;
        std::array<int, 3> plan{};
        char* p = line;
        bool in_plan = false;
        int np = 0;
        while (*p) {
            while (*p == ' ') p++;
            if (*p == '|') {
                in_plan = true;
                p++;
                continue;
            }
            if (*p == '\n' || *p == 0) break;
            char* end = nullptr;
            const long long v = strtoll(p, &end, 10);
            if (end == p) break;
            if (in_plan) {
                if (np < 3) plan[np] = (int)v;
                np++;
            } else {
                key.push_back(v);
            }
            p = end;
        }
        if (np == 3 && !key.empty()) ctx->tune_cache[key] = plan;
    }
    fclose(f);
}

void tune_cache_save(rten_ctx* ctx, const char* path) {
    FILE* f = fopen(path, "w");
    if (!f) return;
    for (const auto& kv : ctx->tune_cache) {
        for (long long v : kv.first) fprintf(f, "%lld ", v);
        fprintf(f, "|");
        for (int v : kv.second) fprintf(f, " %d", v);
        fprintf(f, "\n");
    }
    fclose(f);
}

static rten_status launch_tf32x3(rten_ctx* ctx, const GemmLaunch& L0) {
    GemmLaunch L = L0;
    long long d0 = 0, d0p = 0;
    auto split = [&](const OperandDesc& src, OperandDesc& dst, int role, void* into) -> rten_status {
// ... 100 lines not shown
    }
    void* ws = nullptr;
    if (ws_max) {
        RTB_TRY(ensure_splitk_counters(ctx));
        RTB_TRY(temp_alloc(ctx, ws_max, &ws));
        cudaStreamSynchronize(ctx->stream);
    }
    cudaEvent_t e0, e1;
    cudaEventCreate(&e0);
    cudaEventCreate(&e1);
    auto time_plan = [&](const Plan& x, int n) -> double {
        if (run_plan(ctx, L, q, x, false, ws) != RTEN_OK) return -1.0;
        cudaEventRecord(e0, ctx->stream);
        bool ok = true;
        for (int r = 0; r < n && ok; r++) ok = run_plan(ctx, L, q, x, false, ws) == RTEN_OK;
        cudaEventRecord(e1, ctx->stream);
        if (cudaEventSynchronize(e1) != cudaSuccess || !ok) return -1.0;
        float t = 0.f;
        cudaEventElapsedTime(&t, e0, e1);
        return (double)t / n;
    };
    double best_ms = 1e30;
    int reps = 4;
    std::vector<std::pair<double, size_t>> timed;
    for (size_t i = 0; i < ncand; i++) {
        const Plan& x = cands[i].second;
        double ms = time_plan(x, reps);
        if (ms < 0) continue;
        timed.emplace_back(ms, i);
        if (verbose)
            fprintf(stderr, "[autotune] bn=%d splitk=%d nbuf=%d model=%.0f -> %.2f us\n", x.bn, x.splitk, x.nbuf,
                    cands[i].first, ms * 1e3);
        if (ms < best_ms) {
            best_ms = ms;
            plan = x;
        }
        reps = std::max(4, std::min(32, (int)(0.15 / std::max(best_ms, 1e-3))));
    }
    std::sort(timed.begin(), timed.end());
    best_ms = 1e30;
    for (size_t k = 0; k < std::min<size_t>(3, timed.size()); k++) {
        const Plan& x = cands[timed[k].second].second;
        const double again = time_plan(x, 2 * reps);
        const double ms = again < 0 ? timed[k].first : again;
        if (ms < best_ms) {
            best_ms = ms;
            plan = x;
        }
    }
    for (const auto& s : HALO_SHAPES) {
        const Plan x = halo_plan(s[0], s[1]);
        if (!halo || x.bn > L.N) continue;
        double ms = time_plan(x, reps);
        if (ms > 0 && ms < best_ms * 1.05) ms = time_plan(x, 2 * reps);
        if (verbose && ms > 0) fprintf(stderr, "[autotune] halo bn=%d T=%d -> %.2f us\n", x.bn, x.T, ms * 1e3);
        if (ms > 0 && ms < best_ms * 0.97) {
            best_ms = ms;
            plan = x;
        }
    }
    cudaEventDestroy(e0);
    cudaEventDestroy(e1);
    ctx->tune_cache[tune_key(L, q)] = plan_record(plan);
    return RTEN_OK;
}

rten_status launch_umma_gemm(rten_ctx* ctx, const GemmLaunch& L) {
    const bool verbose = getenv("RTEN_B200_VERBOSE") != nullptr;
    const char* force_bn = getenv("RTEN_B200_FORCE_BN");
    const char* force_sk = getenv("RTEN_B200_FORCE_SPLITK");
    const char* halo_on = getenv("RTEN_B200_HALO");
    const bool halo = L.conv && L.kind == 0 && L.g.kh * L.g.kw > 1 && !L.x3_cb && !L.proj.C && !getenv("RTEN_B200_NO_HALO");
    Prepared q;
    if (L.chain.N2 > 0) {
        if (L.kind != 0 || ctx->f32_mode != RTEN_F32_TF32 || L.x3_cb || getenv("RTEN_B200_NO_CHAIN"))
            return RTEN_ERR_UNSUPPORTED_VALUE;
        RTB_TRY(prepare_launch(ctx, L, q));
        Plan pl;
        pl.bn = 128;
        pl.nbuf = 2;
        return launch_plan(ctx, L, q, pl, verbose);
    }
    if (L.kind == 0 && ctx->f32_mode == RTEN_F32_TF32X3) return launch_tf32x3(ctx, L);
    int hbn, hT;
    if (halo && halo_on && atoi(halo_on) != 0 && halo_model_shape(ctx, L, hbn, hT)) {
        const rten_status hs = run_plan(ctx, L, q, halo_plan(hbn, hT), verbose);
        if (hs != RTEN_ERR_UNSUPPORTED_VALUE) return hs;
    }
    RTB_TRY(prepare_launch(ctx, L, q));
    const bool forced = force_bn || force_sk;
    if (!forced && !ctx->tune_cache.empty()) {
        auto hit = ctx->tune_cache.find(tune_key(L, q));
        if (hit != ctx->tune_cache.end()) {
            const Plan pl = plan_from_record(hit->second);
            PlanShape ps;
            if (pl.halo ? halo && halo_shape_fits(L, pl.bn, pl.T) : plan_shape(q, pl, ps)) return run_plan(ctx, L, q, pl, verbose);
            if (verbose) fprintf(stderr, "[umma_gemm] recorded plan no longer valid for this problem: re-planning\n");
            ctx->tune_cache.erase(hit);
        }
    }
    std::vector<std::pair<double, Plan>> cands;
    enumerate_plans(q, ctx->num_sms, cands);
    if (cands.empty()) return RTEN_ERR_UNSUPPORTED_VALUE;
    Plan plan = cands[0].second;
    if (forced) {
        bool found = false;
        for (const auto& c : cands) {
            const Plan& x = c.second;
            if (force_bn && x.bn != atoi(force_bn)) continue;
            if (force_sk && x.splitk != atoi(force_sk)) continue;
            plan = x;
            found = true;
            break;
        }
        if (!found) {
            ctx->forced_misses++;
            if (verbose) fprintf(stderr, "[umma_gemm] no valid plan matches the forced fields: using the model's choice\n");
            if (getenv("RTEN_B200_FORCE_STRICT"))
                return fail(ctx, RTEN_ERR_INVALID_VALUE, "no launch plan matches the forced RTEN_B200_FORCE_* fields");
        } else {
            ctx->forced_hits++;
        }
    } else if (ctx->autotune) {
        RTB_TRY(autotune(ctx, L, q, cands, halo, verbose, plan));
    }
    return run_plan(ctx, L, q, plan, verbose);
}

}
```

rten_b200/csrc/umma_gemm.h:

```cpp
#pragma once
#include <cuda.h>

#include <cstdint>

#include "common.h"

namespace rtb {

struct OperandDesc {
    const void* base = nullptr;
    int64_t dims[4] = {1, 1, 1, 1};
    int64_t strides[4] = {1, 0, 0, 0};
};

struct EpilogueDesc {
    void* d = nullptr;
    int d_is_i32 = 0;
    int64_t s_z0 = 0, s_z1 = 0, s_row = 0, s_col = 1;
    const float* r = nullptr;
    float r_scale = 1.0f;
    int64_t r_z0 = 0, r_z1 = 0, r_row = 0, r_col = 0;
    const float* bias = nullptr;
    int bias_kind = 0;
    const float* bias2 = nullptr;
    float alpha = 1.0f;
    int act = 0;
    const int32_t* za = nullptr;
    int za_len = 0;
    const uint8_t* za8 = nullptr;
    int za8_signed = 0;
    const int32_t* zb = nullptr;
    int zb_len = 0;
    const int32_t* rowsum = nullptr;
    const int32_t* colsum = nullptr;
    const float* scale = nullptr;
    int scale_len = 0;
    int* range = nullptr;
    const float* scale2 = nullptr;
    float act_alpha = 0.0f, act_beta = 0.0f;
};

struct ConvGeom {
    int B = 0, H = 0, W = 0, C = 0;
    int OH = 0, OW = 0;
    int kh = 1, kw = 1, sy = 1, sx = 1, dy = 1, dx = 1, pt = 0, pl = 0;
};

struct GemmLaunch {
    int kind = 0;
    int a_signed = 0;
    int b_signed = 1;
    int M = 0, N = 0, K = 0;
    int z0 = 1, z1 = 1;
    int conv = 0;
    ConvGeom g;
    OperandDesc a;
    OperandDesc b;
    EpilogueDesc epi;
    void** b_x3_slot = nullptr;
    const void* a_lo_base = nullptr;
    int x3_cb = 0;
    OperandDesc a_lo;
    struct Projection {
        int C = 0;
        int stride = 1;
        OperandDesc a;
        OperandDesc b;
        void** b_x3_slot = nullptr;
        int x3_cb = 0;
        OperandDesc a_lo;
    } proj;
    struct Chain {
        int N2 = 0;
        OperandDesc w;
        const float* bias = nullptr;
        int act = 0;
        OperandDesc z;
    } chain;
};

rten_status launch_umma_gemm(rten_ctx* ctx, const GemmLaunch& L);

bool encode_map(rten_ctx* ctx, CUtensorMap* map, const OperandDesc& od, int esize, bool is_f32, const uint32_t box[4],
                const uint32_t estr[4]);

constexpr int HALO_SHAPES[5][2] = {{32, 1}, {32, 2}, {64, 1}, {64, 2}, {128, 2}};
bool halo_shape_fits(const GemmLaunch& L, int bn, int T);
bool halo_model_shape(rten_ctx* ctx, const GemmLaunch& L, int& bn, int& T);
rten_status launch_umma_halo_conv(rten_ctx* ctx, const GemmLaunch& L, int bn, int T, bool verbose);

void tune_cache_load(rten_ctx* ctx, const char* path);
void tune_cache_save(rten_ctx* ctx, const char* path);

bool tma_compatible(const OperandDesc& od, int esize, int rank);

}
```

rten_b200/csrc/umma_kernel.cuh:

```cuda
#pragma once
#include <cuda.h>
#include <cuda_runtime.h>

#include <cstdint>

#include "math.cuh"
#include "ptx.cuh"
#include "umma_gemm.h"

namespace rtb {

constexpr int BM = 128;
constexpr int KBYTES = 128;
constexpr int A_STAGE_BYTES = BM * KBYTES;
constexpr int ACC_STRIDE = 64;
constexpr int PRODUCER_WARP = 12;
constexpr int NUM_THREADS = 416;
constexpr int STG_BYTES = 128 * 128;
constexpr int MAX_STAGES = 8;

struct FastDiv {
    uint32_t d = 1, mul = 0, shr = 0;
    __host__ void set(int div) {
        d = (uint32_t)(div < 1 ? 1 : div);
        if (d == 1) {
            mul = 0;
            shr = 0;
            return;
        }
        uint32_t lg = 0;
        while ((1ull << lg) < d) lg++;
        const uint32_t p = 31 + lg;
        mul = (uint32_t)(((1ull << p) + d - 1) / d);
        shr = p - 32;
    }
    __device__ __forceinline__ int div(int n) const { return d == 1 ? n : (int)(__umulhi((uint32_t)n, mul) >> shr); }
    __device__ __forceinline__ void divmod(int n, int& q, int& r) const {
        q = div(n);
        r = n - q * (int)d;
    }
};

enum class Epi { Generic, Fast, FastGelu, PlainF32, PlainF32Gelu, PlainI8, PlainI8Gelu };

struct KParams {
    int M, N, K, z0, z1;
    int tiles_m, tiles_n, tiles_total;
    int k_blocks, kelems;
    int bn, stages;
    uint32_t stage_bytes, tx_bytes;
    int sgn;
    int conv;
    int tw, th, tb, tiles_x, tiles_y;
    int OH, OW, Bn;
    int sy, sx, dy, dx, pt, pl, kw, c_blocks;
    int a_bcast0, a_bcast1, b_bcast0, b_bcast1;
    int nbuf;
    int res_tma;
    uint32_t res_tx_bytes;
    int tma_store;
    int splitk;
    int kb_per;
    int units_total;
    int x3_cb;
    int kb_main, kb_proj, s_proj, x3_cb_proj;
    int chain_n2, chain_passes, chain_act;
    const float* chain_bias;
    FastDiv d_tiles_n, d_tiles_m, d_z0, d_tiles_x, d_tiles_y, d_tiles_total, d_c_blocks, d_kw, d_tw, d_th;
    uint32_t* sk_ws;
    int* sk_cnt;
    EpilogueDesc epi;
};

struct TileCoord {
    int n0;
    int m0;
    int z0, z1;
    int ox0, oy0, b0;
};

__device__ __forceinline__ TileCoord decode_tile(const KParams& p, int t) {
    TileCoord c;
    int n_blk, rest, m_blk, z;
    p.d_tiles_n.divmod(t, rest, n_blk);
    p.d_tiles_m.divmod(rest, z, m_blk);
    c.n0 = n_blk * p.bn;
    c.m0 = m_blk * BM;
    p.d_z0.divmod(z, c.z1, c.z0);
    c.ox0 = c.oy0 = c.b0 = 0;
    if (p.conv) {
        int xt, r2, yt, bt;
        p.d_tiles_x.divmod(m_blk, r2, xt);
        p.d_tiles_y.divmod(r2, bt, yt);
        c.ox0 = xt * p.tw;
        c.oy0 = yt * p.th;
        c.b0 = bt * p.tb;
    }
    return c;
}

__device__ __forceinline__ int4 out_coord(const KParams& p, const TileCoord& tc, int col) {
    return p.conv ? make_int4(tc.n0 + col, tc.ox0, tc.oy0, tc.b0) : make_int4(tc.n0 + col, tc.m0, tc.z0, tc.z1);
}

__device__ __forceinline__ void plain_f32_pair(uint32_t& v0, uint32_t& v1, bool res, float2 rr, float2 bb, bool relu) {
    if (res) add_f32x2(v0, v1, rr.x, rr.y);
    add_f32x2(v0, v1, bb.x, bb.y);
    if (relu) {
        v0 = __float_as_uint(fmaxf(__uint_as_float(v0), 0.0f));
        v1 = __float_as_uint(fmaxf(__uint_as_float(v1), 0.0f));
    }
}

__device__ __forceinline__ float column_bias(const EpilogueDesc& e, int n) {
    const float b = __ldg(e.bias + n);
    return e.bias2 ? __fadd_rn(b, __ldg(e.bias2 + n)) : b;
}

__device__ __forceinline__ void bulk_wait_read(int n) {
    switch (n) {
        case 0: asm volatile("cp.async.bulk.wait_group.read 0;" ::: "memory"); break;
        case 1: asm volatile("cp.async.bulk.wait_group.read 1;" ::: "memory"); break;
        case 2: asm volatile("cp.async.bulk.wait_group.read 2;" ::: "memory"); break;
        default: asm volatile("cp.async.bulk.wait_group.read 3;" ::: "memory"); break;
    }
}

__device__ __forceinline__ int f32_to_ordered(float f) {
    const int i = __float_as_int(f);
    return i >= 0 ? i : i ^ 0x7fffffff;
}
__device__ __forceinline__ void range_commit(int* range, float lo, float hi) {
#pragma unroll
    for (int o = 16; o > 0; o >>= 1) {
        lo = fminf(lo, __shfl_xor_sync(0xffffffffu, lo, o));
        hi = fmaxf(hi, __shfl_xor_sync(0xffffffffu, hi, o));
    }
    if ((threadIdx.x & 31) == 0 && lo <= hi) {
        atomicMin(&range[0], f32_to_ordered(lo));
        atomicMax(&range[1], f32_to_ordered(hi));
    }
}

__device__ __noinline__ float4 act4(float4 x, int act, float alpha, float beta) {
    if (act == 2) {
        gelu_ref_x2(x.x, x.y);
        gelu_ref_x2(x.z, x.w);
        return x;
    }
    x.x = apply_act(x.x, act, alpha, beta);
    x.y = apply_act(x.y, act, alpha, beta);
    x.z = apply_act(x.z, act, alpha, beta);
    x.w = apply_act(x.w, act, alpha, beta);
    return x;
}

__device__ __forceinline__ bool splitk_publish(const KParams& p, int t, int ks, int grp, int q, int lane, uint32_t t_acc,
                                               int* flag, uint32_t acc_smem) {
    const int r = q * 32 + lane;
    const int nchunks = p.bn >> 5;
    for (int c0 = grp * 32; c0 < p.bn; c0 += 64) {
        uint32_t v[32];
        acc_ld(acc_smem, t_acc + c0, v);
        uint32_t* w = p.sk_ws + ((((size_t)t * p.splitk + ks) * nchunks + (c0 >> 5)) << 12) + r;
#pragma unroll
        for (int j = 0; j < 32; j++) __stcg(w + j * 128, v[j]);
    }
    __threadfence();
    asm volatile("bar.sync %0, 128;" ::"r"(1 + grp) : "memory");
    if (q == 0 && lane == 0) {
        int* cnt = p.sk_cnt + t * 2 + grp;
        const int old = atomicAdd(cnt, 1);
        const int last = old == p.splitk - 1;
        if (last) *cnt = 0;
        __threadfence();
        *flag = last;
    }
    asm volatile("bar.sync %0, 128;" ::"r"(1 + grp) : "memory");
    return *reinterpret_cast<volatile int*>(flag) != 0;
}

template <int KIND>
__device__ __forceinline__ void splitk_sum(const KParams& p, int t, int c0, int r, uint32_t (&v)[32]) {
    const int nchunks = p.bn >> 5;
    const uint32_t* w = p.sk_ws + ((((size_t)t * p.splitk) * nchunks + (c0 >> 5)) << 12) + r;
    const size_t stride = (size_t)nchunks << 12;
#pragma unroll
    for (int j = 0; j < 32; j++) v[j] = __ldcg(w + j * 128);
#pragma unroll 1
    for (int s = 1; s < p.splitk; s++) {
        w += stride;
#pragma unroll
        for (int j = 0; j < 32; j++) {
            const uint32_t x = __ldcg(w + j * 128);
            if (KIND == 0)
                v[j] = __float_as_uint(__fadd_rn(__uint_as_float(v[j]), __uint_as_float(x)));
            else
                v[j] += x;
        }
    }
}

struct SmemLayout {
    uint8_t* smem;
    uint64_t *full_bar, *empty_bar, *acc_full, *acc_empty, *res_bar, *w_bar;
    int* sk_flag;
    float* bias;
    uint32_t acc_smem;
};

}

#include "umma_epilogue.cuh"

namespace rtb {

template <int KIND, int SGN, int N>
__device__ __forceinline__ void mma_units(const KParams& p, const SmemLayout& L, int worker, int n_workers) {
    const int lane = threadIdx.x & 31;
    const uint32_t smem0 = smem_u32(L.smem);
    uint32_t ring = 0, aphase = 0;
    int stage = 0;
    for (int u = worker, it = 0; u < p.units_total; u += n_workers, it++) {
        const int kb0 = p.d_tiles_total.div(u) * p.kb_per, kb1 = min(p.k_blocks, kb0 + p.kb_per);
        const int acc = it & 1;
        acc_t<KIND> d0[N / 2], d1[N / 2];
#pragma unroll
        for (int i = 0; i < N / 2; i++) d0[i] = d1[i] = 0;
        int prev = -1;
        for (int kb = kb0; kb < kb1; kb++) {
            mbar_wait(&L.full_bar[stage], (ring >> stage) & 1);
            wgmma_fence_operand(d0);
            wgmma_fence_operand(d1);
            wgmma_fence();
            const uint32_t sa = smem0 + stage * p.stage_bytes;
            const uint64_t adesc = make_kmajor_sw128_desc(sa);
            const uint64_t bdesc = make_kmajor_sw128_desc(sa + A_STAGE_BYTES);
#pragma unroll
            for (int k = 0; k < 4; k++) {
                wgmma_k<KIND, SGN, N>(d0, adesc + 2 * k, bdesc + 2 * k);
                wgmma_k<KIND, SGN, N>(d1, adesc + (64 * KBYTES >> 4) + 2 * k, bdesc + 2 * k);
            }
            wgmma_commit();
            wgmma_fence_operand(d0);
            wgmma_fence_operand(d1);
            wgmma_wait<1>();
            if (prev >= 0 && lane == 0) mbar_arrive(&L.empty_bar[prev]);
            prev = stage;
            ring ^= 1u << stage;
            if (++stage == p.stages) stage = 0;
        }
        wgmma_wait<0>();
        wgmma_fence_operand(d0);
        wgmma_fence_operand(d1);
        if (prev >= 0 && lane == 0) mbar_arrive(&L.empty_bar[prev]);
        mbar_wait(&L.acc_empty[acc], ((aphase >> acc) & 1) ^ 1);
        aphase ^= 1u << acc;
        acc_store_frag<N>(L.acc_smem, d0, 0, acc * ACC_STRIDE);
        acc_store_frag<N>(L.acc_smem, d1, 64, acc * ACC_STRIDE);
        mbar_arrive(&L.acc_full[acc]);
    }
}

template <int KIND, int N>
__device__ __forceinline__ void mma_role(const KParams& p, const SmemLayout& L, int worker, int n_workers) {
    if (KIND == 0) mma_units<KIND, 0, N>(p, L, worker, n_workers);
    else if (p.sgn == 0) mma_units<KIND, 0, N>(p, L, worker, n_workers);
    else if (p.sgn == 1) mma_units<KIND, 1, N>(p, L, worker, n_workers);
    else if (p.sgn == 2) mma_units<KIND, 2, N>(p, L, worker, n_workers);
    else mma_units<KIND, 3, N>(p, L, worker, n_workers);
}

struct TmaMaps {
    CUtensorMap a, b, d, r, a2, a_proj, b_proj, a2_proj, w2, z;
};

__device__ __forceinline__ void prefetch_maps(const TmaMaps& m, const KParams& p) {
    tma_prefetch_desc(&m.a);
    tma_prefetch_desc(&m.b);
    if (p.tma_store) tma_prefetch_desc(&m.d);
    if (p.res_tma) tma_prefetch_desc(&m.r);
    if (p.x3_cb) tma_prefetch_desc(&m.a2);
    if (p.kb_proj) {
        tma_prefetch_desc(&m.a_proj);
        tma_prefetch_desc(&m.b_proj);
        if (p.x3_cb_proj) tma_prefetch_desc(&m.a2_proj);
    }
}

template <bool CHAIN = false>
__device__ __forceinline__ void producer_role(const KParams& p, const TmaMaps& m, const SmemLayout& L, int worker,
                                              int n_workers) {
    uint8_t* smem = L.smem;
    uint64_t* empty_bar = L.empty_bar;
    uint32_t ring = 0;
    int stage = 0;
    const uint32_t smem0 = smem_u32(smem);
    const uint32_t full0 = smem_u32(L.full_bar);
    for (int u = worker; u < p.units_total; u += n_workers) {
      for (int pass = 0; pass < (CHAIN ? p.chain_passes : 1); pass++) {
        int t, ks;
        p.d_tiles_total.divmod(u, ks, t);
        const int kb0 = ks * p.kb_per, kb1 = min(p.k_blocks, kb0 + p.kb_per);
        TileCoord tc = decode_tile(p, t);
        if (CHAIN) tc.n0 += pass * p.bn;
        bool proj = kb0 >= p.kb_main;
        int x3 = proj ? p.x3_cb_proj : p.x3_cb;
        int tap = 0, cb = kb0 - p.kb_main, ky, kx;
        if (!proj) p.d_c_blocks.divmod(kb0, tap, cb);
        p.d_kw.divmod(tap, ky, kx);
        int seg = 0, sblk = p.conv ? cb : kb0;
        if (x3)
            while (sblk >= x3) {
                sblk -= x3;
                seg++;
            }
        if (u == worker && pass == 0) {
            pdl_wait();
            if (CHAIN && elect_one()) {
                const int cb2 = p.N / 32;
                const uint32_t wbytes = (uint32_t)(p.chain_n2 * KBYTES);
                uint8_t* w2 = smem + (size_t)p.stages * p.stage_bytes;
                mbar_expect_tx(L.w_bar, cb2 * wbytes);
                for (int c = 0; c < cb2; c++) tma_load_4d(w2 + c * wbytes, &m.w2, L.w_bar, 32 * c, 0, 0, 0);
            }
            if (CHAIN) __syncwarp();
        }
        for (int kb = kb0; kb < kb1; kb++) {
            if (kb == p.kb_main) {
                proj = true;
                x3 = p.x3_cb_proj;
                cb = sblk = seg = 0;
            }
            mbar_wait(&empty_bar[stage], ((ring >> stage) & 1) ^ 1);
            if (elect_one()) {
                const uint32_t fb = full0 + stage * 8;
                mbar_expect_tx_u32(fb, p.tx_bytes);
                const uint32_t sa = smem0 + stage * p.stage_bytes;
                const uint32_t sb = sa + A_STAGE_BYTES;
                const bool lo = x3 && seg == 0;
                if (proj) {
                    const int c0 = cb * p.kelems;
                    tma_load_4d_u32(sa, lo ? &m.a2_proj : &m.a_proj, fb, x3 ? sblk * p.kelems : c0, tc.ox0 * p.s_proj,
                                    tc.oy0 * p.s_proj, tc.b0);
                    tma_load_4d_u32(sb, &m.b_proj, fb, c0, tc.n0, 0, 0);
                } else if (p.conv) {
                    const int c0 = cb * p.kelems;
                    const int ca = x3 ? sblk * p.kelems : c0;
                    tma_load_4d_u32(sa, lo ? &m.a2 : &m.a, fb, ca, tc.ox0 * p.sx - p.pl + kx * p.dx, tc.oy0 * p.sy - p.pt + ky * p.dy, tc.b0);
                    tma_load_4d_u32(sb, &m.b, fb, c0, tc.n0, tap, 0);
                } else {
                    const int k0 = kb * p.kelems;
                    const int ka = x3 ? sblk * p.kelems : k0;
                    tma_load_4d_u32(sa, lo ? &m.a2 : &m.a, fb, ka, tc.m0, p.a_bcast0 ? 0 : tc.z0, p.a_bcast1 ? 0 : tc.z1);
                    tma_load_4d_u32(sb, &m.b, fb, k0, tc.n0, p.b_bcast0 ? 0 : tc.z0, p.b_bcast1 ? 0 : tc.z1);
                }
            }
            if (x3 && ++sblk == x3) {
                sblk = 0;
                seg = seg == 2 ? 0 : seg + 1;
            }
            if (++cb == p.c_blocks && !proj) {
                cb = 0;
                tap++;
                if (++kx == p.kw) {
                    kx = 0;
                    ky++;
                }
            }
            __syncwarp();
            ring ^= 1u << stage;
            if (++stage == p.stages) stage = 0;
        }
      }
    }
}

constexpr int SMEM_FIXED_BYTES = 1024  + 4096  + ACC_SMEM_BYTES;
static_assert(ACC_SMEM_BYTES % 1024 == 0, "operand stages must stay 1024-B aligned");
static_assert(2 * ACC_STRIDE <= ACC_COLS, "two accumulator stages");

__device__ __forceinline__ SmemLayout carve_smem(uint8_t* smem_raw) {
    uint8_t* base = reinterpret_cast<uint8_t*>((reinterpret_cast<uintptr_t>(smem_raw) + 1023) & ~uintptr_t(1023));
    SmemLayout L;
    L.full_bar = reinterpret_cast<uint64_t*>(base);
    L.empty_bar = L.full_bar + MAX_STAGES;
    L.acc_full = L.empty_bar + MAX_STAGES;
    L.acc_empty = L.acc_full + 2;
    L.res_bar = L.acc_empty + 2;
    L.sk_flag = reinterpret_cast<int*>(L.res_bar + 8) + 2;
    L.bias = reinterpret_cast<float*>(base + 1024);
    L.acc_smem = smem_u32(base + 4096);
    L.smem = base + 4096 + ACC_SMEM_BYTES;
    return L;
}

__device__ __forceinline__ void kernel_setup(const SmemLayout& L) {
    const int warp = threadIdx.x >> 5;
    const int lane = threadIdx.x & 31;
    if (warp == PRODUCER_WARP) {
// ... 337 lines not shown
```

rten_b200/graphs.py:

```python
from __future__ import annotations

import math
from dataclasses import dataclass, field
from typing import Callable, List, Optional

import numpy as np

from . import ops as O



@dataclass
class ConvSpec:
    w: np.ndarray
    b: np.ndarray
    stride: int
    pad: int


@dataclass
class Bottleneck:
    c1: ConvSpec
    c2: ConvSpec
    c3: ConvSpec
# ... 32 lines not shown
    return ResNet50Spec(stem, blocks, fc_w, fc_b)


def resnet50_flops(spec: ResNet50Spec, hw: int = 224) -> float:

    def out(h, k, s, p):
        return (h + 2 * p - k) // s + 1

    total = 0.0
    h = out(hw, 7, 2, 3)
    total += 2.0 * spec.stem.w.shape[0] * h * h * 3 * 49
    h = out(h, 3, 2, 1)
    for b in spec.blocks:
        for c, hin in ((b.c1, h), (b.c2, h)):
            o, i, k, _ = c.w.shape
            ho = out(hin, k, c.stride, c.pad)
            total += 2.0 * o * ho * ho * i * k * k
        h2 = out(h, 3, b.c2.stride, 1)
        o, i, _, _ = b.c3.w.shape
        total += 2.0 * o * h2 * h2 * i
        if b.down is not None:
            o, i, _, _ = b.down.w.shape
            total += 2.0 * o * h2 * h2 * i
        h = h2
    total += 2.0 * spec.fc_w.shape[0] * spec.fc_w.shape[1]
    return total


class ResNet50Runner:

    def __init__(self, ctx: O.Context, spec: ResNet50Spec, fuse: bool = True, chain: bool = True):
        self.ctx, self.spec, self.fuse, self.chain = ctx, spec, fuse, chain
        self._convs = {}

        def prep(c: ConvSpec):
            op = O.Conv(1, (1, 1), (c.pad, c.pad, c.pad, c.pad), (c.stride, c.stride))
            w = ctx.to_device(c.w)
            self._convs[id(c)] = (op, w, ctx.to_device(c.b), op.prepack(ctx, 1, w))

        prep(spec.stem)
        for b in spec.blocks:
            for c in (b.c1, b.c2, b.c3, b.down):
                if c is not None:
                    prep(c)
        self.fc_w = ctx.to_device(spec.fc_w)
        self.fc_b = ctx.to_device(spec.fc_b)
        self.maxpool = O.MaxPool((3, 3), (1, 1, 1, 1), (2, 2))
        self.gap = O.GlobalAveragePool()
        self.fc = O.Gemm(1.0, 1.0, False, True)
        self.relu, self.add = O.Relu(), O.Add()

    def _conv(self, c: ConvSpec, x, relu: bool, residual=None):
        op, w, b, pk = self._convs[id(c)]
        if self.fuse:
            op.activation = O.ACT_RELU if relu else O.ACT_NONE
            return op.run(self.ctx, x, w, b, packed_w=pk, residual=residual)
        op.activation = O.ACT_NONE
        y = op.run(self.ctx, x, w, b, packed_w=pk)
        if residual is not None:
            y = self.add.run(self.ctx, y, residual)
        if relu:
            y = self.relu.run(self.ctx, y, in_place=True)
        return y

    def _conv_projected(self, c: ConvSpec, t, down: ConvSpec, x):
        op, w, b, pk = self._convs[id(c)]
        dop, dw, db, dpk = self._convs[id(down)]
        op.activation = O.ACT_RELU
        return op.run_projected(self.ctx, t, w, b, packed_w=pk, proj=dop, x_proj=x, w_proj=dw, bias_proj=db, packed_w_proj=dpk)

    def _conv_chained(self, b: Bottleneck, t, x, nxt: ConvSpec):
        op, w, bias, pk = self._convs[id(b.c3)]
        nop, nw, nb, npk = self._convs[id(nxt)]
        op.activation = nop.activation = O.ACT_RELU
        kw = dict(nxt=nop, w_next=nw, bias_next=nb, packed_w_next=npk)
        if b.down is None:
            return op.run_chained(self.ctx, t, w, bias, packed_w=pk, residual=x, **kw)
        dop, dw, db, dpk = self._convs[id(b.down)]
        return op.run_chained(self.ctx, t, w, bias, packed_w=pk, proj=dop, x_proj=x, w_proj=dw, bias_proj=db,
                              packed_w_proj=dpk, **kw)

    def run(self, x: O.DeviceTensor) -> O.DeviceTensor:
        s = self.spec
        y = self._conv(s.stem, x, True)
        y = self.maxpool.run(self.ctx, y)
        t1 = None
        for i, b in enumerate(s.blocks):
            if self.fuse and self.chain and i + 1 < len(s.blocks):
                t = t1 if t1 is not None else self._conv(b.c1, y, True)
                t = self._conv(b.c2, t, True)
                y, t1 = self._conv_chained(b, t, y, s.blocks[i + 1].c1)
                continue
            if self.fuse and b.down is not None:
                t = self._conv(b.c1, y, True)
                t = self._conv(b.c2, t, True)
                y = self._conv_projected(b.c3, t, b.down, y)
                continue
            ident = y if b.down is None else self._conv(b.down, y, False)
            t = t1 if t1 is not None else self._conv(b.c1, y, True)
            t = self._conv(b.c2, t, True)
            y = self._conv(b.c3, t, True, residual=ident)
        p = self.gap.run(self.ctx, y)
        return self.fc.run(self.ctx, p.reshape(p.shape[0], p.shape[1]), self.fc_w, self.fc_b)




def load_mnist_weights(path: str) -> dict:
    z = np.load(path)
    return {k[2:]: z[k] for k in z.files if k.startswith("w:")}


class MnistRunner:
    def __init__(self, ctx: O.Context, weights: dict, fuse: bool = True):
        self.ctx, self.fuse = ctx, fuse
        dev = ctx.to_device
        self.w = {k: dev(v) for k, v in weights.items()}
        self.c1 = O.Conv(1, (1, 1), (1, 1, 1, 1), (1, 1))
        self.c2 = O.Conv(1, (1, 1), (1, 1, 1, 1), (1, 1))
        self.pw = O.Conv(1, (1, 1), (0, 0, 0, 0), (1, 1))
        self.pool = O.MaxPool((2, 2), (0, 0, 0, 0), (2, 2))
        self.relu, self.gap, self.fc = O.Relu(), O.GlobalAveragePool(), O.Gemm(1.0, 1.0, False, True)

    def _conv(self, op, x, name):
        if self.fuse:
            op.activation = O.ACT_RELU
            return op.run(self.ctx, x, self.w[name + ".weight"], self.w[name + ".bias"])
        op.activation = O.ACT_NONE
        return self.relu.run(self.ctx, op.run(self.ctx, x, self.w[name + ".weight"], self.w[name + ".bias"]), in_place=True)

    def run(self, x: O.DeviceTensor) -> O.DeviceTensor:
        ctx = self.ctx
        y = self.pool.run(ctx, self._conv(self.c1, x, "conv1"))
        y = self.pool.run(ctx, self._conv(self.c2, y, "conv2"))
        y = self._conv(self.pw, y, "pw")
        p = self.gap.run(ctx, y)
        return self.fc.run(ctx, p.reshape(p.shape[0], p.shape[1]), self.w["fc.weight"], self.w["fc.bias"])




@dataclass
class QConvSpec:
    wq: np.ndarray
    w_scale: np.ndarray
    b: np.ndarray
    stride: int
    pad: int


@dataclass
class ResNet50Int8Spec:
    stem: QConvSpec
    blocks: List[Bottleneck]
    fc_w: np.ndarray
    fc_b: np.ndarray


def _quantize_sym(w: np.ndarray, axis=None):
    amax = np.max(np.abs(w), axis=axis, keepdims=axis is not None).astype(np.float32)
    scale = (np.maximum(amax, np.float32(1e-12)) / np.float32(64.0)).astype(np.float32)
    q = np.clip(np.rint(w / scale), -64, 64).astype(np.int8)
    return q, scale


def quantize_resnet50(spec: ResNet50Spec) -> ResNet50Int8Spec:
    def qc(c: ConvSpec):
        q, s = _quantize_sym(c.w)
# ... 518 lines not shown
```

rten_b200/ops.py:

```python
from __future__ import annotations

import ctypes as C
from typing import Optional, Sequence

import numpy as np

from . import _lib
from ._lib import (RTEN_DEVICE_HOST, RTEN_F32, RTEN_I8, RTEN_I32, RTEN_U8, RtenActivation, RtenAttentionParams, RtenConvParams,
                   RtenConvTransposeParams, RtenGqaParams, RtenMhaParams, RtenResizeParams, RtenTensor, RtenRnnParams)

_NP2RT = {np.dtype(np.float32): RTEN_F32, np.dtype(np.int32): RTEN_I32, np.dtype(np.int8): RTEN_I8,
          np.dtype(np.uint8): RTEN_U8}
_RT2NP = {v: k for k, v in _NP2RT.items()}

ACT_NONE, ACT_RELU, ACT_GELU, ACT_GELU_TANH = 0, 1, 2, 3
ACT_SIGMOID, ACT_SILU, ACT_HARD_SIGMOID, ACT_HARD_SWISH = 4, 5, 6, 7


class OpError(Exception):

    def __init__(self, status: int, msg: str):
        self.status = status
        self.kind = _lib.STATUS_NAMES.get(status, str(status))
        self.msg = msg
# ... 475 lines not shown
                                         C.byref(y) if 0 in outputs else None, C.byref(yh) if 1 in outputs else None,
                                         C.byref(yc) if 2 in outputs else None))
        return tuple(A.wrap(o, None) if i in outputs else None for i, o in enumerate((y, yh, yc)))


def _conv_params(padding, groups, strides, dilations) -> RtenConvParams:
    p = RtenConvParams()
    if isinstance(padding, str):
        if padding.lower() != "same":
            raise OpError(5, "unknown padding mode")
        p.auto_pad_same = 1
    else:
        pads = list(padding)
        if len(pads) == 2:
            pads = [pads[0], pads[1], 0, 0]
        if len(pads) != 4:
            raise OpError(5, "Wrong number of pad values")
        for i in range(4):
            p.pads[i] = int(pads[i])
    p.groups = int(groups)
    p.n_strides = len(strides)
    p.n_dilations = len(dilations)
    for i in range(min(2, len(strides))):
        p.strides[i] = int(strides[i])
    for i in range(min(2, len(dilations))):
        p.dilations[i] = int(dilations[i])
    return p


def _activation(activation) -> RtenActivation:
    kind, alpha, beta = tuple(activation) if isinstance(activation, (tuple, list)) else (activation, 0.2, 0.5)
    return RtenActivation(int(kind), float(alpha), float(beta))


class Conv:

    def __init__(self, groups=1, dilations=(1, 1), padding=(0, 0, 0, 0), strides=(1, 1), activation=ACT_NONE):
        self.groups, self.dilations, self.padding, self.strides = groups, tuple(dilations), padding, tuple(strides)
        self.activation = activation

    def prepack(self, ctx, index, value):
        if index != 1:
            return None
        A = _Args(ctx)
        h = C.c_void_p()
        ctx.check(ctx.lib.rten_b200_prepack_conv_weight(ctx.handle, A.t(value), self.groups, C.byref(h)))
        return Packed(ctx, h)

    def run(self, ctx, x, w, bias=None, packed_w: Optional[Packed] = None, residual=None, out=None):
        A = _Args(ctx)
        o = A.out(out)
        p = _conv_params(self.padding, self.groups, self.strides, self.dilations)
        act = _activation(self.activation)
        ctx.check(ctx.lib.rten_b200_conv2d_act(ctx.handle, A.t(x), A.t(w), _ph(packed_w), A.t(bias), C.byref(p),
                                               A.t(residual), C.byref(act), C.byref(o)))
        return A.wrap(o, out)

    def run_projected(self, ctx, x, w, bias=None, packed_w: Optional[Packed] = None, *, proj: "Conv", x_proj, w_proj,
                      bias_proj=None, packed_w_proj: Optional[Packed] = None, out=None):
        A = _Args(ctx)
        o = A.out(out)
        p = _conv_params(self.padding, self.groups, self.strides, self.dilations)
        pp = _conv_params(proj.padding, proj.groups, proj.strides, proj.dilations)
        ctx.check(ctx.lib.rten_b200_conv2d_projected(ctx.handle, A.t(x), A.t(w), _ph(packed_w), A.t(bias), C.byref(p),
                                                     A.t(x_proj), A.t(w_proj), _ph(packed_w_proj), A.t(bias_proj),
                                                     C.byref(pp), self.activation, C.byref(o)))
        return A.wrap(o, out)

    def run_chained(self, ctx, x, w, bias=None, packed_w: Optional[Packed] = None, residual=None, *, nxt: "Conv", w_next,
                    bias_next=None, packed_w_next: Optional[Packed] = None, proj: Optional["Conv"] = None, x_proj=None,
                    w_proj=None, bias_proj=None, packed_w_proj: Optional[Packed] = None, out=None, out_next=None):
        A = _Args(ctx)
        o, o2 = A.out(out), A.out(out_next)
        p = _conv_params(self.padding, self.groups, self.strides, self.dilations)
        pn = _conv_params(nxt.padding, nxt.groups, nxt.strides, nxt.dilations)
        pp = _conv_params(proj.padding, proj.groups, proj.strides, proj.dilations) if proj is not None else None
        ctx.check(ctx.lib.rten_b200_conv2d_chained(ctx.handle, A.t(x), A.t(w), _ph(packed_w), A.t(bias), C.byref(p),
                                                   A.t(residual), A.t(x_proj), A.t(w_proj), _ph(packed_w_proj),
                                                   A.t(bias_proj), C.byref(pp) if pp is not None else None,
                                                   self.activation, A.t(w_next), _ph(packed_w_next), A.t(bias_next),
                                                   C.byref(pn), nxt.activation, C.byref(o), C.byref(o2)))
        return A.wrap(o, out), A.wrap(o2, out_next)


def _conv_transpose_params(padding, groups, strides, dilations, output_padding) -> RtenConvTransposeParams:
    p = RtenConvTransposeParams()
    if isinstance(padding, str):
        if padding.lower() != "same":
            raise OpError(5, "unknown padding mode")
        p.auto_pad_same = 1
    else:
        pads = list(padding)
        p.n_pads = len(pads)
        for i in range(min(4, len(pads))):
            p.pads[i] = int(pads[i])
    p.groups = int(groups)
    for arr, vals, n in ((p.strides, strides, "n_strides"), (p.dilations, dilations, "n_dilations"),
                         (p.output_padding, output_padding or (), "n_output_padding")):
        setattr(p, n, len(vals))
        for i in range(min(2, len(vals))):
            arr[i] = int(vals[i])
    return p


class ConvTranspose:

    def __init__(self, groups=1, dilations=(1, 1), padding=(0, 0, 0, 0), strides=(1, 1), output_padding=None):
        self.groups, self.dilations, self.padding, self.strides = groups, tuple(dilations), padding, tuple(strides)
        self.output_padding = None if output_padding is None else tuple(output_padding)

    def _params(self):
        return _conv_transpose_params(self.padding, self.groups, self.strides, self.dilations, self.output_padding)

    def prepack(self, ctx, index, value):
        if index != 1:
            return None
        A = _Args(ctx)
        h = C.c_void_p()
        p = self._params()
        ctx.check(ctx.lib.rten_b200_prepack_conv_transpose_weight(ctx.handle, A.t(value), C.byref(p), C.byref(h)))
        return Packed(ctx, h)

    def run(self, ctx, x, w, bias=None, packed_w: Optional[Packed] = None, out=None):
        A = _Args(ctx)
        o = A.out(out)
        p = self._params()
        ctx.check(ctx.lib.rten_b200_conv_transpose(ctx.handle, A.t(x), A.t(w), _ph(packed_w), A.t(bias), C.byref(p),
                                                   C.byref(o)))
        return A.wrap(o, out)


class ConvInteger(Conv):

    def run(self, ctx, x, w, x_zero_point=None, w_zero_point=None, packed_w: Optional[Packed] = None, out=None):
        A = _Args(ctx)
        o = A.out(out)
        p = _conv_params(self.padding, self.groups, self.strides, self.dilations)
        ctx.check(ctx.lib.rten_b200_conv_integer(ctx.handle, A.t(x), A.t(w), _ph(packed_w), A.t(x_zero_point),
                                                 A.t(w_zero_point), None, C.byref(p), C.byref(o)))
        return A.wrap(o, out)


class ConvIntegerToFloat(Conv):

    def run(self, ctx, x, w, x_zero_point, w_zero_point, scale, packed_w: Optional[Packed] = None, out=None,
            bias=None, residual=None, scale_b=None, out_range=None):
        if scale is None:
            raise OpError(4, "missing inputs")
        A = _Args(ctx)
        o = A.out(out)
        p = _conv_params(self.padding, self.groups, self.strides, self.dilations)
        ctx.check(ctx.lib.rten_b200_conv_integer_ex(ctx.handle, A.t(x), A.t(w), _ph(packed_w), A.t(x_zero_point),
                                                    A.t(w_zero_point), A.t(scale), A.t(scale_b), C.byref(p), A.t(bias),
                                                    A.t(residual), self.activation, A.t(out_range), C.byref(o)))
        return A.wrap(o, out)


class Softmax:

    def __init__(self, axis=-1, flush_nans_to_zero=False):
        self.axis, self.flush_nans_to_zero = axis, flush_nans_to_zero

    def run(self, ctx, x, in_place=False):
        A = _Args(ctx)
        into = x if (in_place and isinstance(x, DeviceTensor)) else None
        o = A.out(into)
# ... 374 lines not shown
```

Before: 17230.

## Fuse ResNet stem conv with following max-pool in UMMA GEMM epilogue

Adds a conv2d_pooled entry point that runs the stem 7x7 conv and applies the 3x3/2 max-pool inside the GEMM epilogue. Tiles become row strips, and a per-group ring of three rows in shared memory holds horizontally pooled results that are then reduced vertically. The goal is to avoid writing and re-reading the full-resolution stem activation and to drop a separate maxpool launch. In exchange it changes tile scheduling so each worker walks consecutive strip rows, uses extra shared memory, and restricts which tile shapes can be used. When conditions are not met, it falls back to a temporary buffer followed by a separate pool.

```diff
diff --git a/include/rten_b200.h b/include/rten_b200.h
--- a/include/rten_b200.h
+++ b/include/rten_b200.h
@@ -143,6 +143,10 @@
                                      const rten_packed* packed_w_next_or_null, const rten_tensor* bias_next_or_null,
                                      const rten_conv_params* p_next, int activation_next, rten_tensor* out,
                                      rten_tensor* out_next);
+rten_status rten_b200_conv2d_pooled(rten_ctx* ctx, const rten_tensor* x, const rten_tensor* w,
+                                    const rten_packed* packed_w_or_null, const rten_tensor* bias_or_null,
+                                    const rten_conv_params* p, int activation, const int32_t kernel[2],
+                                    const int32_t pads[4], const int32_t strides[2], rten_tensor* out);
 typedef struct {
     int32_t pads[4];
     int32_t auto_pad_same;
diff --git a/rten_b200/_lib.py b/rten_b200/_lib.py
--- a/rten_b200/_lib.py
+++ b/rten_b200/_lib.py
@@ -127,6 +127,8 @@
     "rten_b200_conv2d_chained": (C.c_int, [_vp, _TP, _TP, _vp, _TP, C.POINTER(RtenConvParams), _TP, _TP, _TP, _vp, _TP,
                                            C.POINTER(RtenConvParams), C.c_int, _TP, _vp, _TP, C.POINTER(RtenConvParams),
                                            C.c_int, _TP, _TP]),
+    "rten_b200_conv2d_pooled": (C.c_int, [_vp, _TP, _TP, _vp, _TP, C.POINTER(RtenConvParams), C.c_int,
+                                          C.POINTER(C.c_int32), C.POINTER(C.c_int32), C.POINTER(C.c_int32), _TP]),
     "rten_b200_conv_transpose": (C.c_int, [_vp, _TP, _TP, _vp, _TP, C.POINTER(RtenConvTransposeParams), _TP]),
     "rten_b200_prepack_conv_transpose_weight": (C.c_int, [_vp, _TP, C.POINTER(RtenConvTransposeParams), C.POINTER(_vp)]),
     "rten_b200_conv_integer": (C.c_int, [_vp, _TP, _TP, _vp, _TP, _TP, _TP, C.POINTER(RtenConvParams), _TP]),
diff --git a/rten_b200/csrc/api_conv.cu b/rten_b200/csrc/api_conv.cu
--- a/rten_b200/csrc/api_conv.cu
+++ b/rten_b200/csrc/api_conv.cu
@@ -36,6 +36,7 @@
     const rten_tensor* out_range = nullptr;
     const void* x_lo = nullptr;
     bool cache_x3 = true;
+    const GemmLaunch::Pool* pool = nullptr;
 };
 
 rten_status pack_conv_weight(rten_ctx* ctx, const rten_tensor* w, int esize, void* dst) {
@@ -269,7 +270,14 @@
 
     const int out_dtype = (A.kind == 1 && !A.scale) ? RTEN_I32 : RTEN_F32;
     rten_tensor ov;
-    RTB_TRY(out_like(sc, out, out_dtype, x, one_d, B, O, OH, OW, &ov));
+    if (A.pool) {
+        if (one_d || A.kind != 0 || groups != 1 || A.residual || A.act > RTEN_ACT_RELU || B * O * OH * OW == 0 ||
+            !(x.strides[1] == 1 && C > 1) || (out->data && out->strides[1] != 1))
+            return RTEN_ERR_UNSUPPORTED_VALUE;
+        RTB_TRY(out_like(sc, out, out_dtype, x, one_d, B, O, A.pool->PH, A.pool->PW, &ov));
+    } else {
+        RTB_TRY(out_like(sc, out, out_dtype, x, one_d, B, O, OH, OW, &ov));
+    }
     if (B * O * OH * OW == 0) return RTEN_OK;
 
     const int esize = A.kind == 0 ? 4 : 1;
@@ -319,6 +327,7 @@
     const bool pointwise_1x1 = kh == 1 && kw == 1 && (pt | pb | pl | pr) == 0 && groups == 1 && strides[0] == 1 &&
                                strides[1] == 1 && dil[0] == 1 && dil[1] == 1;
     if (C == O && groups == C && !pointwise_1x1) {
+        if (A.pool) return RTEN_ERR_UNSUPPORTED_VALUE;
         DepthwiseParams d;
         d.x_dtype = x.dtype;
         d.w_dtype = w.dtype;
@@ -489,9 +498,11 @@
         }
         L.b = packed_weight(wsm, kb, O, kh);
         epilogue(L.epi, 0);
+        if (A.pool) L.pool = *A.pool;
         const rten_status st = launch_umma_gemm(ctx, L);
         if (st != RTEN_ERR_UNSUPPORTED_VALUE) return st;
     }
+    if (A.pool && !implicit_ok) return RTEN_ERR_UNSUPPORTED_VALUE;
 
     for (int g = 0; g < groups; g++) {
         GemmLaunch L;
@@ -535,11 +546,13 @@
                 if (const rten_status st = launch_umma_gemm(ctx, R)) return fail(ctx, st, "conv window-sum GEMM could not be launched");
                 e.rowsum = rs;
             }
+            if (A.pool) L.pool = *A.pool;
             const rten_status st = launch_umma_gemm(ctx, L);
             if (st != RTEN_ERR_UNSUPPORTED_VALUE) {
                 RTB_TRY(st);
                 continue;
             }
+            if (A.pool) return st;
         }
         const int64_t Kd = kh * kw * Cg;
         const int64_t kpad = round_up(Kd, 16 / esize);
@@ -1320,13 +1333,9 @@
     return sc.finish(conv_core(sc, A, out));
 }
 
-static rten_status pool2d(rten_ctx* ctx, const rten_tensor* x, const int32_t kernel[2], const int32_t pads[4],
-                          const int32_t strides[2], bool average, int count_include_pad, rten_tensor* out) {
-    RTB_TRY(check_ctx(ctx));
-    if (!x || !out) return fail(ctx, RTEN_ERR_MISSING_INPUTS, "missing inputs");
-    if (x->dtype != RTEN_F32) return fail(ctx, RTEN_ERR_UNSUPPORTED_TYPE, "unsupported type");
-    if (x->ndim != 4) return fail(ctx, RTEN_ERR_INVALID_VALUE, "input must have 4 dims (NCHW)");
-    OpScope sc(ctx);
+static rten_status pool_core(OpScope& sc, const rten_tensor* x, const int32_t kernel[2], const int32_t pads[4],
+                             const int32_t strides[2], bool average, int count_include_pad, rten_tensor* out) {
+    rten_ctx* ctx = sc.ctx;
     rten_tensor xv, ov;
     RTB_TRY(sc.in(x, &xv));
     int64_t OH = 0, OW = 0, p0, p1;
@@ -1356,8 +1365,74 @@
     p.ys_h = ov.strides[2];
     p.ys_w = ov.strides[3];
     p.channels_fastest = ov.strides[1] == 1;
-    return sc.finish(average ? launch_avgpool(ctx, (const float*)xv.data, (float*)ov.data, p, count_include_pad)
-                             : launch_maxpool(ctx, (const float*)xv.data, (float*)ov.data, p));
+    return average ? launch_avgpool(ctx, (const float*)xv.data, (float*)ov.data, p, count_include_pad)
+                   : launch_maxpool(ctx, (const float*)xv.data, (float*)ov.data, p);
+}
+
+static rten_status pool2d(rten_ctx* ctx, const rten_tensor* x, const int32_t kernel[2], const int32_t pads[4],
+                          const int32_t strides[2], bool average, int count_include_pad, rten_tensor* out) {
+    RTB_TRY(check_ctx(ctx));
+    if (!x || !out) return fail(ctx, RTEN_ERR_MISSING_INPUTS, "missing inputs");
+    if (x->dtype != RTEN_F32) return fail(ctx, RTEN_ERR_UNSUPPORTED_TYPE, "unsupported type");
+    if (x->ndim != 4) return fail(ctx, RTEN_ERR_INVALID_VALUE, "input must have 4 dims (NCHW)");
+    OpScope sc(ctx);
+    return sc.finish(pool_core(sc, x, kernel, pads, strides, average, count_include_pad, out));
+}
+
+rten_status rten_b200_conv2d_pooled(rten_ctx* ctx, const rten_tensor* x, const rten_tensor* w, const rten_packed* pw,
+                                    const rten_tensor* bias, const rten_conv_params* p, int activation,
+                                    const int32_t kernel[2], const int32_t pads[4], const int32_t strides[2],
+                                    rten_tensor* out) {
+    RTB_TRY(check_ctx(ctx));
+    if (!x || !w || !p || !kernel || !pads || !strides || !out) return fail(ctx, RTEN_ERR_MISSING_INPUTS, "missing inputs");
+    if (x->dtype != RTEN_F32 || w->dtype != RTEN_F32 || (bias && bias->dtype != RTEN_F32))
+        return fail(ctx, RTEN_ERR_UNSUPPORTED_TYPE, "unsupported type");
+    if (activation < RTEN_ACT_NONE || activation > RTEN_ACT_GELU_TANH) return fail(ctx, RTEN_ERR_INVALID_VALUE, "unknown activation");
+    if (x->ndim != 4) return fail(ctx, RTEN_ERR_INVALID_VALUE, "input must have 4 dims (NCHW)");
+    OpScope sc(ctx);
+    ConvArgs A{};
+    A.kind = 0;
+    A.x = x;
+    A.w = w;
+    A.pw = pw;
+    A.bias = bias;
+    A.p = p;
+    A.act = activation;
+    ConvShape S;
+    RTB_TRY(conv_shape(sc, A, S));
+    int64_t PH = 0, PW = 0, p0, p1;
+    RTB_TRY(axis_out(ctx, S.OH, kernel[0], strides[0], false, pads[0], pads[2], 1, &PH, &p0, &p1));
+    RTB_TRY(axis_out(ctx, S.OW, kernel[1], strides[1], false, pads[1], pads[3], 1, &PW, &p0, &p1));
+    GemmLaunch::Pool pp;
+    pp.kh = kernel[0];
+    pp.kw = kernel[1];
+    pp.sy = strides[0];
+    pp.sx = strides[1];
+    pp.pt = pads[0];
+    pp.pl = pads[1];
+    pp.PH = (int)PH;
+    pp.PW = (int)PW;
+    const bool one = pp.kh <= 3 && pp.kw <= 3 && pp.sy <= 2 && pp.sx <= 2 && pads[0] < pp.kh && pads[1] < pp.kw &&
+                     pads[2] < pp.kh && pads[3] < pp.kw && PH > 0 && PW > 0 && PH < (1 << 20) && PW <= 128 &&
+                     (!out->data || out->device >= 0) && !getenv("RTEN_B200_NO_POOL");
+    if (one) {
+        A.pool = &pp;
+        const rten_status st = conv_core(sc, A, out);
+        if (st != RTEN_ERR_UNSUPPORTED_VALUE) return sc.finish(st);
+        A.pool = nullptr;
+    }
+    const OutLayout l = layout_like(S.x, false, S.B, S.O, S.OH, S.OW);
+    rten_tensor y{};
+    y.dtype = RTEN_F32;
+    y.ndim = 4;
+    y.device = ctx->device;
+    for (int i = 0; i < 4; i++) {
+        y.shape[i] = l.shape[i];
+        y.strides[i] = l.strides[i];
+    }
+    RTB_TRY(temp_alloc(ctx, (size_t)std::max<int64_t>(S.B * S.O * S.OH * S.OW, 1) * 4, &y.data));
+    RTB_TRY(conv_core(sc, A, &y));
+    return sc.finish(pool_core(sc, &y, kernel, pads, strides, false, 0, out));
 }
 
 rten_status rten_b200_max_pool(rten_ctx* ctx, const rten_tensor* x, const int32_t kernel[2], const int32_t pads[4],
diff --git a/rten_b200/csrc/umma_epilogue.cuh b/rten_b200/csrc/umma_epilogue.cuh
--- a/rten_b200/csrc/umma_epilogue.cuh
+++ b/rten_b200/csrc/umma_epilogue.cuh
@@ -381,8 +381,71 @@
     }
 };
 
+__device__ __forceinline__ int pool_slot_items(const KParams& p) { return 8 * (p.PW + 1); }
+__device__ __forceinline__ float4* pool_ring(const KParams& p, const SmemLayout& L, int grp) {
+    return reinterpret_cast<float4*>(L.smem + (size_t)p.stages * p.stage_bytes) + grp * 3 * pool_slot_items(p);
+}
+
+__device__ __forceinline__ float4 pool_act4(const KParams& p, uint32_t acc_smem, int acc_col, int row, float4 bb) {
+    uint32_t w[4];
+#pragma unroll
+    for (int u = 0; u < 4; u++)
+        asm volatile("ld.shared.b32 %0, [%1];" : "=r"(w[u]) : "r"(acc_smem + (((acc_col + u) * ACC_LD + row) << 2)) : "memory");
+    plain_f32_pair(w[0], w[1], false, make_float2(0.f, 0.f), make_float2(bb.x, bb.y), p.epi.act == 1);
+    plain_f32_pair(w[2], w[3], false, make_float2(0.f, 0.f), make_float2(bb.z, bb.w), p.epi.act == 1);
+    return make_float4(__uint_as_float(w[0]), __uint_as_float(w[1]), __uint_as_float(w[2]), __uint_as_float(w[3]));
+}
+
+__device__ __forceinline__ float4 max_first(float4 x, float4 m) {
+    m.x = x.x > m.x ? x.x : m.x;
+    m.y = x.y > m.y ? x.y : m.y;
+    m.z = x.z > m.z ? x.z : m.z;
+    m.w = x.w > m.w ? x.w : m.w;
+    return m;
+}
+
+__device__ __forceinline__ void pool_chunk(const KParams& p, const SmemLayout& L, int grp, int t, int acc_col0, int nbase) {
+    if (nbase >= p.N) return;
+    int j, n_blk, b, py0;
+    pool_strip(p, t, j, n_blk, b, py0);
+    const int i0 = threadIdx.x & 127;
+    const float* bias_s = L.bias + grp * 128;
+    const int pw1 = p.PW + 1, n_slot = pool_slot_items(p), n_items = 8 * p.PW;
+    const float ninf = __int_as_float(0xff800000);
+    float4* const ring = pool_ring(p, L, grp);
+    float4* const slot = ring + (j % 3) * n_slot;
+    for (int i = i0; i < n_items; i += 128) {
+        const int c = i / p.PW, px = i - c * p.PW;
+        const float4 bb = *reinterpret_cast<const float4*>(bias_s + 4 * c);
+        float4 m = make_float4(ninf, ninf, ninf, ninf);
+        for (int kx = 0; kx < p.pool_kw; kx++) {
+            const int ix = px * p.pool_sx - p.pool_pl + kx;
+            if (ix < 0 || ix >= p.OW) continue;
+            m = max_first(pool_act4(p, L.acc_smem, acc_col0 + 4 * c, ix, bb), m);
+        }
+        slot[c * pw1 + px] = m;
+    }
+    const int jl = j - (p.pool_kh - 1);
+    if (jl < 0 || jl % p.pool_sy) return;
+    const int py = py0 + jl / p.pool_sy;
+    group_sync(grp);
+    if (py >= p.PH) return;
+    const EpilogueDesc& e = p.epi;
+    float* out = reinterpret_cast<float*>(e.d) + (long long)b * e.s_z0 + (long long)py * e.s_row + nbase;
+    for (int i = i0; i < n_items; i += 128) {
+        const int px = i >> 3, c = i & 7;
+        float4 m = make_float4(ninf, ninf, ninf, ninf);
+        for (int ky = 0; ky < p.pool_kh; ky++) {
+            const int oy = py * p.pool_sy - p.pool_pt + ky;
+            if (oy < 0 || oy >= p.OH) continue;
+            m = max_first(ring[((jl + ky) % 3) * n_slot + c * pw1 + px], m);
+        }
+        *reinterpret_cast<float4*>(out + (long long)px * e.s_z1 + 4 * c) = m;
+    }
+}
+
 template <int KIND, Epi E>
-using EpiOps = std::conditional_t<E == Epi::Generic, GenericEpi<KIND>,
+using EpiOps =std::conditional_t<E == Epi::Generic, GenericEpi<KIND>,
                std::conditional_t<E == Epi::Fast || E == Epi::FastGelu, FastEpi<KIND, E == Epi::FastGelu>,
                std::conditional_t<E == Epi::PlainF32 || E == Epi::PlainF32Gelu, PlainF32Epi<E == Epi::PlainF32Gelu>,
                                   PlainI8Epi<E == Epi::PlainI8Gelu>>>>;
@@ -405,7 +468,7 @@
     Ops ops(p, L, grp);
     uint32_t ci = 0;
     uint32_t aphase = 0, rphase = 0;
-    for (int u = worker, it = 0; u < p.units_total; u += n_workers, it++) {
+    for (int u = first_unit(p, worker), it = 0; u < p.units_total; u = next_unit(p, u, n_workers), it++) {
         int t = u, ks = 0;
         if (splitk > 1) p.d_tiles_total.divmod(u, ks, t);
         const int acc = it & 1;
@@ -434,43 +497,52 @@
             const TileCoord tc = (E == Epi::Fast || E == Epi::FastGelu) ? tc0 : decode_tile(p, t);
             ops.row(p, tc, r);
             if (const int c0 = grp * 32, k = 0; c0 < p.bn) {
-                uint32_t v[32];
-                if (splitk > 1)
-                    splitk_sum<KIND>(p, t, c0, r, v);
-                else
-                    acc_ld(L.acc_smem, t_row + c0, v);
-                const int nbase = tc.n0 + c0;
-                const int bcur = ci % nbuf;
-                uint8_t* stg = stg0 + bcur * STG_BYTES;
-                uint8_t* rowp = stg + r * 128;
-                if (p.res_tma) {
-                    mbar_wait(&L.res_bar[grp * 4 + bcur], (rphase >> bcur) & 1);
-                    rphase ^= 1u << bcur;
-                }
-                ops.math(p, v, k, nbase, rowp, sw);
-                if (tma_store && nbuf == 1) {
-                    if (issuer) bulk_wait_read(0);
-                    group_sync(grp);
-                }
-#pragma unroll
-                for (int j = 0; j < 8; j++)
-                    *reinterpret_cast<uint4*>(staged_chunk(rowp, sw, j)) = make_uint4(v[4 * j], v[4 * j + 1], v[4 * j + 2], v[4 * j + 3]);
-                ops.staged(p, nbase, rowp, sw);
-                if (tma_store) {
-                    if (issuer && !p.res_tma && nbuf > 1) bulk_wait_read(nbuf - 2);
-                    fence_proxy_async();
-                    group_sync(grp);
-                    if (issuer) {
-                        const int4 x = out_coord(p, tc, c0);
-                        tma_store_4d(tma_d, stg, x.x, x.y, x.z, x.w);
-                        asm volatile("cp.async.bulk.commit_group;" ::: "memory");
-                    }
-                } else if (ops.row_ok) {
-                    if constexpr (Ops::kDirectStore) {
-                        uint32_t* dptr = reinterpret_cast<uint32_t*>(e.d) + ops.d_off;
+                bool pooled = false;
+                if constexpr (E == Epi::PlainF32) {
+                    if (p.pool_T) {
+                        pool_chunk(p, L, grp, t, acc * ACC_STRIDE + c0, tc.n0 + c0);
+                        pooled = true;
+                    }
+                }
+                if (!pooled) {
+                    uint32_t v[32];
+                    if (splitk > 1)
+                        splitk_sum<KIND>(p, t, c0, r, v);
+                    else
+                        acc_ld(L.acc_smem, t_row + c0, v);
+                    const int nbase = tc.n0 + c0;
+                    const int bcur = ci % nbuf;
+                    uint8_t* stg = stg0 + bcur * STG_BYTES;
+                    uint8_t* rowp = stg + r * 128;
+                    if (p.res_tma) {
+                        mbar_wait(&L.res_bar[grp * 4 + bcur], (rphase >> bcur) & 1);
+                        rphase ^= 1u << bcur;
+                    }
+                    ops.math(p, v, k, nbase, rowp, sw);
+                    if (tma_store && nbuf == 1) {
+                        if (issuer) bulk_wait_read(0);
+                        group_sync(grp);
+                    }
+#pragma unroll
+                    for (int j = 0; j < 8; j++)
+                        *reinterpret_cast<uint4*>(staged_chunk(rowp, sw, j)) = make_uint4(v[4 * j], v[4 * j + 1], v[4 * j + 2], v[4 * j + 3]);
+                    ops.staged(p, nbase, rowp, sw);
+                    if (tma_store) {
+                        if (issuer && !p.res_tma && nbuf > 1) bulk_wait_read(nbuf - 2);
+                        fence_proxy_async();
+                        group_sync(grp);
+                        if (issuer) {
+                            const int4 x = out_coord(p, tc, c0);
+                            tma_store_4d(tma_d, stg, x.x, x.y, x.z, x.w);
+                            asm volatile("cp.async.bulk.commit_group;" ::: "memory");
+                        }
+                    } else if (ops.row_ok) {
+                        if constexpr (Ops::kDirectStore) {
+                            uint32_t* dptr = reinterpret_cast<uint32_t*>(e.d) + ops.d_off;
 #pragma unroll 1
-                        for (int j = 0; j < 32 && nbase + j < p.N; j++)
-                            dptr[(long long)(nbase + j) * e.s_col] = *staged_word(rowp, sw, j);
+                            for (int j = 0; j < 32 && nbase + j < p.N; j++)
+                                dptr[(long long)(nbase + j) * e.s_col] = *staged_word(rowp, sw, j);
+                        }
                     }
                 }
                 ci++;
diff --git a/rten_b200/csrc/umma_gemm.cu b/rten_b200/csrc/umma_gemm.cu
--- a/rten_b200/csrc/umma_gemm.cu
+++ b/rten_b200/csrc/umma_gemm.cu
@@ -118,6 +118,7 @@
     int tma_store, res_tma;
     int wide;
     int chain_bytes;
+    int pool_bytes;
     int step;
     int esize, kelems;
 };
@@ -181,9 +182,10 @@
         if (pl.bn % 32 || (long long)(pl.splitk - 1) * ps.kb_per >= p.k_blocks) return false;
         if (ps.tiles * 2 > SK_CNT_INTS) return false;
     }
-    ps.n_stg = 2 * pl.nbuf;
+    ps.n_stg = q.pool_bytes ? 0 : 2 * pl.nbuf;
     ps.stage_bytes = A_STAGE_BYTES + pl.bn * KBYTES;
-    ps.stages = is_wide(pl.bn) ? wide_stages(ps.stage_bytes, q.chain_bytes) : std::min(MAX_STAGES, smem_budget_for(ps.n_stg) / ps.stage_bytes);
+    ps.stages = is_wide(pl.bn) ? wide_stages(ps.stage_bytes, q.chain_bytes)
+                               : std::min(MAX_STAGES, (smem_budget_for(ps.n_stg) - q.pool_bytes) / ps.stage_bytes);
     if (ps.stages < 2) return false;
     return true;
 }
@@ -261,6 +263,10 @@
     if (L.conv) {
         const ConvGeom& g = L.g;
         pick_conv_tile(g, p.tw, p.th, p.tb);
+        if (L.pool.kh > 0 && g.OW <= 128) {
+            p.tw = g.OW;
+            p.th = p.tb = 1;
+        }
         p.tiles_x = (g.OW + p.tw - 1) / p.tw;
         p.tiles_y = (g.OH + p.th - 1) / p.th;
         int tiles_b = (g.B + p.tb - 1) / p.tb;
@@ -378,6 +384,49 @@
             return RTEN_ERR_UNSUPPORTED_VALUE;
         q.chain_bytes = L.N / 32 * c.N2 * KBYTES;
     }
+    q.pool_bytes = 0;
+    if (L.pool.kh > 0) {
+        const GemmLaunch::Pool& pp = L.pool;
+        const ConvGeom& g = L.g;
+        const uintptr_t d_addr = reinterpret_cast<uintptr_t>(e.d);
+        if (!L.conv || L.kind != 0 || L.N % 32 || g.OW > 128 || g.OW * g.sx > 256 || pp.kh < 1 || pp.kh > 3 ||
+            pp.kw < 1 || pp.kw > 3 || pp.sy < 1 || pp.sy > 2 || pp.sx < 1 || pp.sx > 2 || pp.pt < 0 || pp.pl < 0 ||
+            pp.pt >= pp.kh || pp.pl >= pp.kw || pp.PH < 1 || pp.PW < 1 || pp.PW > 128 || e.s_col != 1 || (d_addr & 15) ||
+            (e.s_z0 | e.s_row | e.s_z1) % 4 || e.alpha != 1.0f || e.r || e.range || e.bias2 || e.act > 1 ||
+            e.bias_kind == 2 || L.proj.C > 0 || L.chain.N2 > 0)
+            return RTEN_ERR_UNSUPPORTED_VALUE;
+        const int bn = L.N % 64 == 0 ? 64 : 32;
+        const long long per_image = (long long)((L.N + bn - 1) / bn) * g.B;
+        long long best = -1;
+        int S = 1;
+        for (int s = 1; s <= pp.PH; s++) {
+            const long long strips = per_image * ((pp.PH + s - 1) / s);
+            const long long rows = (strips + ctx->num_sms - 1) / ctx->num_sms * ((long long)(s - 1) * pp.sy + pp.kh);
+            if (best < 0 || rows <= best) {
+                best = rows;
+                S = s;
+            }
+        }
+        p.pool_S = S;
+        p.pool_T = (S - 1) * pp.sy + pp.kh;
+        p.pool_kh = pp.kh;
+        p.pool_kw = pp.kw;
+        p.pool_sy = pp.sy;
+        p.pool_sx = pp.sx;
+        p.pool_pt = pp.pt;
+        p.pool_pl = pp.pl;
+        p.PH = pp.PH;
+        p.PW = pp.PW;
+        const int strips = (pp.PH + S - 1) / S;
+        p.d_pool_T.set(p.pool_T);
+        p.d_pool_strips.set(strips);
+        const long long tiles_m = (long long)g.B * strips * p.pool_T;
+        if (tiles_m > 0x7FFFFFFFll) return RTEN_ERR_UNSUPPORTED_VALUE;
+        p.tiles_m = (int)tiles_m;
+        q.tma_store = q.res_tma = 0;
+        q.wide = 0;
+        q.pool_bytes = 2 * 3 * 8 * (pp.PW + 1) * 16;
+    }
     return RTEN_OK;
 }
 
@@ -453,7 +502,7 @@
         p.res_tma = 0;
         m.r = m.a;
     }
-    const Epi epi = pick_epilogue(L, p.tma_store, p.res_tma, p.splitk);
+    const Epi epi = p.pool_T ? Epi::PlainF32 : pick_epilogue(L, p.tma_store, p.res_tma, p.splitk);
     if (epi == Epi::Generic && (L.kind == 1 || L.epi.act > 1)) p.res_tma = 0;
     if (q.chain_bytes) {
         const GemmLaunch::Chain& c = L.chain;
@@ -467,14 +516,19 @@
         p.chain_bias = c.bias;
     }
 
-    if (verbose)
-        fprintf(stderr, "[umma_gemm] kind=%d conv=%d M=%d N=%d K=%d kb=%d kb_proj=%d tiles_m=%d bn=%d splitk=%d units=%d stages=%d tma_store=%d res_tma=%d nbuf=%d box=%dx%dx%d epi=%s%s\n",
+    if (verbose) {
+        char pool[96] = "";
+        if (p.pool_T)
+            snprintf(pool, sizeof(pool), " pooled=%dx%d/%dx%d S=%d T=%d", p.pool_kh, p.pool_kw, p.pool_sy, p.pool_sx,
+                     p.pool_S, p.pool_T);
+        fprintf(stderr, "[umma_gemm] kind=%d conv=%d M=%d N=%d K=%d kb=%d kb_proj=%d tiles_m=%d bn=%d splitk=%d units=%d stages=%d tma_store=%d res_tma=%d nbuf=%d box=%dx%dx%d epi=%s%s%s\n",
                 L.kind, L.conv, L.M, L.N, L.K, p.k_blocks, p.kb_proj, p.tiles_m, p.bn, p.splitk, p.units_total, p.stages,
                 p.tma_store, p.res_tma, p.nbuf, p.tw, p.th, p.tb, epi_name(epi),
-                p.chain_n2 == 64 ? " chain=64" : p.chain_n2 == 128 ? " chain=128" : "");
+                p.chain_n2 == 64 ? " chain=64" : p.chain_n2 == 128 ? " chain=128" : "", pool);
+    }
     if ((is_wide(p.bn) || p.kb_proj || L.epi.bias2) && !is_plain_f32(epi)) return RTEN_ERR_UNSUPPORTED_VALUE;
     const size_t smem_bytes = (size_t)p.stages * p.stage_bytes + q.chain_bytes +
-                              (is_wide(p.bn) ? WIDE_SMEM_FIXED_BYTES : ps.n_stg * STG_BYTES + SMEM_FIXED_BYTES);
+                              (is_wide(p.bn) ? WIDE_SMEM_FIXED_BYTES : ps.n_stg * STG_BYTES + SMEM_FIXED_BYTES) + q.pool_bytes;
     using Kernel = void (*)(TmaMaps, KParams);
     static const Kernel narrow[2][7] = {
         {umma_gemm_kernel<0, Epi::Generic>, umma_gemm_kernel<0, Epi::Fast>, umma_gemm_kernel<0, Epi::FastGelu>,
@@ -488,7 +542,8 @@
                                                    : umma_wide_kernel<Epi::PlainF32>;
 
     const int threads = is_wide(p.bn) ? WIDE_THREADS : NUM_THREADS;
-    return launch(ctx, "umma_gemm launch", kern, {std::min(p.units_total, ctx->num_sms), threads, smem_bytes, 227 * 1024, true}, m, p);
+    const int workers = p.pool_T ? p.units_total / p.pool_T : p.units_total;
+    return launch(ctx, "umma_gemm launch", kern, {std::min(workers, ctx->num_sms), threads, smem_bytes, 227 * 1024, true}, m, p);
 }
 
 static std::vector<long long> tune_key(const GemmLaunch& L, const Prepared& q) {
@@ -755,6 +810,23 @@
         return launch_plan(ctx, L, q, pl, verbose);
     }
     if (L.kind == 0 && ctx->f32_mode == RTEN_F32_TF32X3) return launch_tf32x3(ctx, L);
+    if (L.pool.kh > 0) {
+        if (getenv("RTEN_B200_NO_POOL")) return RTEN_ERR_UNSUPPORTED_VALUE;
+        GemmLaunch Lc = L;
+        Lc.pool = GemmLaunch::Pool();
+        int tw, th, tb;
+        pick_conv_tile(L.g, tw, th, tb);
+        const long long plain_tiles = (long long)((L.g.OW + tw - 1) / tw) * ((L.g.OH + th - 1) / th) * ((L.g.B + tb - 1) / tb);
+        if (!L.conv || plain_tiles < 2ll * ctx->num_sms) return RTEN_ERR_UNSUPPORTED_VALUE;
+        if (L.kind == 0 && L.g.kh * L.g.kw > 1 && !L.x3_cb && !getenv("RTEN_B200_NO_HALO"))
+            for (const auto& hs : HALO_SHAPES)
+                if (halo_shape_fits(Lc, hs[0], hs[1])) return RTEN_ERR_UNSUPPORTED_VALUE;
+        RTB_TRY(prepare_launch(ctx, L, q));
+        Plan pl;
+        pl.bn = L.N % 64 == 0 ? 64 : 32;
+        pl.nbuf = 1;
+        return launch_plan(ctx, L, q, pl, verbose);
+    }
     int hbn, hT;
     if (halo && halo_on && atoi(halo_on) != 0 && halo_model_shape(ctx, L, hbn, hT)) {
         const rten_status hs = run_plan(ctx, L, q, halo_plan(hbn, hT), verbose);
diff --git a/rten_b200/csrc/umma_gemm.h b/rten_b200/csrc/umma_gemm.h
--- a/rten_b200/csrc/umma_gemm.h
+++ b/rten_b200/csrc/umma_gemm.h
@@ -77,6 +77,10 @@
         int act = 0;
         OperandDesc z;
     } chain;
+    struct Pool {
+        int kh = 0, kw = 0, sy = 1, sx = 1, pt = 0, pl = 0;
+        int PH = 0, PW = 0;
+    } pool;
 };
 
 rten_status launch_umma_gemm(rten_ctx* ctx, const GemmLaunch& L);
diff --git a/rten_b200/csrc/umma_kernel.cuh b/rten_b200/csrc/umma_kernel.cuh
--- a/rten_b200/csrc/umma_kernel.cuh
+++ b/rten_b200/csrc/umma_kernel.cuh
@@ -66,6 +66,8 @@
     int kb_main, kb_proj, s_proj, x3_cb_proj;
     int chain_n2, chain_passes, chain_act;
     const float* chain_bias;
+    int pool_T, pool_S, pool_kh, pool_kw, pool_sy, pool_sx, pool_pt, pool_pl, PH, PW;
+    FastDiv d_pool_T, d_pool_strips;
     FastDiv d_tiles_n, d_tiles_m, d_z0, d_tiles_x, d_tiles_y, d_tiles_total, d_c_blocks, d_kw, d_tw, d_th;
     uint32_t* sk_ws;
     int* sk_cnt;
@@ -79,8 +81,32 @@
     int ox0, oy0, b0;
 };
 
+__device__ __forceinline__ void pool_strip(const KParams& p, int t, int& j, int& n_blk, int& b, int& py0) {
+    int s, rest, sb;
+    p.d_pool_T.divmod(t, s, j);
+    p.d_tiles_n.divmod(s, rest, n_blk);
+    p.d_pool_strips.divmod(rest, b, sb);
+    py0 = sb * p.pool_S;
+}
+
+__device__ __forceinline__ int first_unit(const KParams& p, int worker) { return p.pool_T ? worker * p.pool_T : worker; }
+__device__ __forceinline__ int next_unit(const KParams& p, int u, int n_workers) {
+    if (!p.pool_T) return u + n_workers;
+    return p.d_pool_T.div(u + 1) * p.pool_T == u + 1 ? u + 1 + (n_workers - 1) * p.pool_T : u + 1;
+}
+
 __device__ __forceinline__ TileCoord decode_tile(const KParams& p, int t) {
     TileCoord c;
+    if (p.pool_T) {
+        int j, n_blk, b, py0;
+        pool_strip(p, t, j, n_blk, b, py0);
+        c.n0 = n_blk * p.bn;
+        c.m0 = c.z0 = c.z1 = 0;
+        c.ox0 = 0;
+        c.oy0 = py0 * p.pool_sy - p.pool_pt + j;
+        c.b0 = b;
+        return c;
+    }
     int n_blk, rest, m_blk, z;
     p.d_tiles_n.divmod(t, rest, n_blk);
     p.d_tiles_m.divmod(rest, z, m_blk);
@@ -221,7 +247,7 @@
     const uint32_t smem0 = smem_u32(L.smem);
     uint32_t ring = 0, aphase = 0;
     int stage = 0;
-    for (int u = worker, it = 0; u < p.units_total; u += n_workers, it++) {
+    for (int u = first_unit(p, worker), it = 0; u < p.units_total; u = next_unit(p, u, n_workers), it++) {
         const int kb0 = p.d_tiles_total.div(u) * p.kb_per, kb1 = min(p.k_blocks, kb0 + p.kb_per);
         const int acc = it & 1;
         acc_t<KIND> d0[N / 2], d1[N / 2];
@@ -297,7 +323,7 @@
     int stage = 0;
     const uint32_t smem0 = smem_u32(smem);
     const uint32_t full0 = smem_u32(L.full_bar);
-    for (int u = worker; u < p.units_total; u += n_workers) {
+    for (int u = first_unit(p, worker); u < p.units_total; u = next_unit(p, u, n_workers)) {
       for (int pass = 0; pass < (CHAIN ? p.chain_passes : 1); pass++) {
         int t, ks;
         p.d_tiles_total.divmod(u, ks, t);
@@ -315,7 +341,7 @@
                 sblk -= x3;
                 seg++;
             }
-        if (u == worker && pass == 0) {
+        if (u == first_unit(p, worker) && pass == 0) {
             pdl_wait();
             if (CHAIN && elect_one()) {
                 const int cb2 = p.N / 32;
diff --git a/rten_b200/graphs.py b/rten_b200/graphs.py
--- a/rten_b200/graphs.py
+++ b/rten_b200/graphs.py
@@ -138,8 +138,12 @@
 
     def run(self, x: O.DeviceTensor) -> O.DeviceTensor:
         s = self.spec
-        y = self._conv(s.stem, x, True)
-        y = self.maxpool.run(self.ctx, y)
+        if self.fuse:
+            op, w, b, pk = self._convs[id(s.stem)]
+            op.activation = O.ACT_RELU
+            y = op.run_pooled(self.ctx, x, w, b, packed_w=pk, pool=self.maxpool)
+        else:
+            y = self.maxpool.run(self.ctx, self._conv(s.stem, x, True))
         t1 = None
         for i, b in enumerate(s.blocks):
             if self.fuse and self.chain and i + 1 < len(s.blocks):
diff --git a/rten_b200/ops.py b/rten_b200/ops.py
--- a/rten_b200/ops.py
+++ b/rten_b200/ops.py
@@ -581,6 +581,17 @@
                                                    C.byref(pn), nxt.activation, C.byref(o), C.byref(o2)))
         return A.wrap(o, out), A.wrap(o2, out_next)
 
+    def run_pooled(self, ctx, x, w, bias=None, packed_w: Optional[Packed] = None, *, pool: "MaxPool", out=None):
+        A = _Args(ctx)
+        o = A.out(out)
+        p = _conv_params(self.padding, self.groups, self.strides, self.dilations)
+        k = (C.c_int32 * 2)(*pool.kernel_size)
+        pp = (C.c_int32 * 4)(*pool.padding)
+        s = (C.c_int32 * 2)(*pool.strides)
+        ctx.check(ctx.lib.rten_b200_conv2d_pooled(ctx.handle, A.t(x), A.t(w), _ph(packed_w), A.t(bias), C.byref(p),
+                                                  self.activation, k, pp, s, C.byref(o)))
+        return A.wrap(o, out)
+
 
 def _conv_transpose_params(padding, groups, strides, dilations, output_padding) -> RtenConvTransposeParams:
     p = RtenConvTransposeParams()
```

Result: faster. 17600, median of 6 (+2.2%).
